# RaphaelHaddad/Real-Time-Brain-Inspired-Video-Memory

Hardware: NVIDIA B200
Metric: queries_per_sec_top10_384d (higher is better)
Workload: dtype tf32

## Files before the change

include/vidmem.h:

```cpp
#ifndef VIDMEM_H_
#define VIDMEM_H_

#include <stddef.h>
#include <stdint.h>

#ifdef __cplusplus
extern "C" {
#endif

#define VM_ABI_VERSION 1

typedef enum vm_status {
    VM_OK = 0,
    VM_ERR_BADARG = -1,
    VM_ERR_OOM = -2,
    VM_ERR_CUDA = -3,
    VM_ERR_NCCL = -4,
    VM_ERR_OVERFLOW = -5,
    VM_ERR_UNSUPPORTED = -6,
    VM_ERR_STATE = -7
} vm_status;

typedef enum vm_dtype { VM_F32 = 0, VM_BF16 = 1, VM_F64 = 2 } vm_dtype;
typedef enum vm_mem { VM_MEM_HOST = 0, VM_MEM_DEVICE = 1 } vm_mem;

typedef enum vm_score_mode { VM_SCORE_RAW = 0, VM_SCORE_NEO4J = 1 } vm_score_mode;

typedef enum vm_sum_mode { VM_SUM_NAIVE = 0, VM_SUM_NEUMAIER = 1 } vm_sum_mode;

enum {
    VM_FLAG_ASYNC = 1,
    VM_FLAG_FORCE_EXACT = 2,
    VM_FLAG_FORCE_SIMT = 4,
    VM_FLAG_FORCE_TC = 8,
    VM_FLAG_TIMING = 16,
    VM_FLAG_NO_SPLIT = 32,
    VM_FLAG_SPLIT = 64
};

typedef struct vm_store vm_store;
typedef struct vm_comm vm_comm;

typedef struct vm_topk_stats {
    int32_t scan_kernel;
    int32_t scan_launches;
    int32_t uncertified;
    int32_t candidates;
    int32_t scan_ctas;
    int32_t scan_stages;
    int32_t full_rescans;
    int32_t scan_variant;
} vm_topk_stats;

int vm_version(void);
const char *vm_last_error(void);
int vm_device_info(int device, int *sm_count, int *cc_major, int *cc_minor, size_t *total_mem);

int vm_store_create(vm_store **out, int device, int dim, int dtype, int64_t capacity);
int vm_store_attach(vm_store **out, int device, int dim, int dtype, int64_t capacity, void *rows_dev,
                    float *inv_norms_dev);
int vm_store_create_exact(vm_store **out, int device, int dim, int shadow_dtype, int64_t capacity);
int vm_store_attach_exact(vm_store **out, int device, int dim, int shadow_dtype, int64_t capacity, void *rows_dev,
                          float *inv_norms_dev, double *rows_exact_dev);
int vm_store_create_growable(vm_store **out, int device, int dim, int dtype, int exact, int64_t initial_capacity,
                             int64_t max_capacity);
int vm_store_reserve(vm_store *s, int64_t capacity);
int64_t vm_store_max_capacity(const vm_store *s);
size_t vm_store_resident_bytes(const vm_store *s);
void *vm_store_rows_ptr(const vm_store *s);
float *vm_store_inv_norms_ptr(const vm_store *s);
double *vm_store_rows_exact_ptr(const vm_store *s);
int vm_store_destroy(vm_store *s);
int64_t vm_store_size(const vm_store *s);
int64_t vm_store_capacity(const vm_store *s);
int vm_store_dim(const vm_store *s);
int vm_store_ld(const vm_store *s);
int vm_ld(int dim);

int vm_store_append(vm_store *s, const void *rows, int src_dtype, int src_mem, int64_t n, int64_t *first_row,
                    void *stream);
int vm_store_update(vm_store *s, int64_t row0, const void *rows, int src_dtype, int src_mem, int64_t n,
                    void *stream);
int vm_store_invalidate(vm_store *s, const int64_t *rows_host, int64_t n, void *stream);
int vm_store_set_size(vm_store *s, int64_t n, int64_t recompute_from_row, void *stream);
int vm_store_clear(vm_store *s);
int vm_store_last_scan_ms(vm_store *s, float *ms);
int vm_store_avg_scan_ms(vm_store *s, float *ms, int *calls);

typedef struct vm_store_counters {
    int64_t batches;
    int64_t queries;
    int64_t uncertified;
    int64_t band_settled;
    int64_t collect_settled;
    int64_t full_rescans;
    int64_t bound_violations;
} vm_store_counters;
int vm_store_read_counters(vm_store *s, vm_store_counters *out, int reset);

int vm_store_band_keys(vm_store *s, int nq_cap, int64_t *kept_per_query, int64_t *spilled_per_query, int *nq_out);

int vm_topk(vm_store *s, const void *queries, int q_dtype, int q_mem, int nq, int k, double min_score,
            int score_mode, int sum_mode, int flags, int64_t *out_idx, double *out_score, int32_t *out_count,
            int out_mem, vm_topk_stats *stats, void *stream);

int vm_topk_sharded(vm_store *s, vm_comm *comm, int64_t row_offset, const void *queries, int q_dtype, int q_mem,
                    int nq, int k, double min_score, int score_mode, int sum_mode, int flags, int64_t *out_idx,
                    double *out_score, int32_t *out_count, int out_mem, vm_topk_stats *stats, void *stream);

int vm_merge_topk_lists(int device, const int64_t *idx_dev, const double *score_dev, const int32_t *count_dev,
                        int nlists, int nq, int k, int64_t *out_idx_dev, double *out_score_dev,
                        int32_t *out_count_dev, void *stream);

size_t vm_topk_packed_bytes(int nq, int k);
int vm_merge_topk_packed(int device, const void *packed_dev, int nlists, int nq, int k, int64_t *out_idx_dev,
                         double *out_score_dev, int32_t *out_count_dev, void *stream);

int vm_merge_max_by_id(int device, const int64_t *idx_dev, const double *score_dev, const int32_t *count_dev,
                       int nq, int k, int k2, int64_t *out_idx_dev, double *out_score_dev,
                       int32_t *out_count_dev, void *stream);

int vm_cosine_pairs(int device, const void *a, const void *b, int dtype, int mem, int64_t n, int dim, int zero_rule,
                    int sum_mode, double *out, int out_mem, void *stream);

int vm_pairs_above(int device, const void *x_dev, int dtype, int64_t n, int dim, float threshold, int64_t cap,
                   int64_t *out_i_dev, int64_t *out_j_dev, float *out_score_dev, int64_t *out_count_dev, int part,
                   int nparts, int flags, void *stream);

int vm_pairs_above_sharded(vm_comm *comm, void *x_dev, int dtype, int64_t n, int dim, float threshold, int64_t cap,
                           int64_t *out_i_dev, int64_t *out_j_dev, float *out_score_dev, int64_t *out_count_dev,
                           int root, int flags, void *stream);

int vm_comm_unique_id(void *out128);
int vm_comm_init_rank(vm_comm **out, int device, int nranks, int rank, const void *id128);
int vm_comm_destroy(vm_comm *c);
size_t vm_comm_exchange_bytes(void);
int vm_comm_attach_peer_buffers(vm_comm *c, void *const *bufs, int nranks);
int vm_comm_nranks(const vm_comm *c);
int vm_comm_rank(const vm_comm *c);

int vm_synth_fill(int device, void *rows_dev, int dtype, uint64_t seed, int64_t row0, int64_t n, int dim,
                  uint64_t dup_period, void *stream);

#ifdef __cplusplus
}
#endif
#endif
```

real-time-brain-inspired-video-memory_b200/_lib.py:

```python
from __future__ import annotations

import ctypes as C
import os
import sys

HERE = os.path.dirname(os.path.abspath(__file__))
LIB_PATH = os.environ.get("VIDMEM_LIB", os.path.join(HERE, "libvidmem.so"))

VM_OK = 0
VM_ERR_BADARG, VM_ERR_OOM, VM_ERR_CUDA, VM_ERR_NCCL, VM_ERR_OVERFLOW, VM_ERR_UNSUPPORTED, VM_ERR_STATE = -1, -2, -3, -4, -5, -6, -7
VM_F32, VM_BF16, VM_F64 = 0, 1, 2
VM_MEM_HOST, VM_MEM_DEVICE = 0, 1
VM_SCORE_RAW, VM_SCORE_NEO4J = 0, 1
VM_SUM_NAIVE, VM_SUM_NEUMAIER = 0, 1
VM_FLAG_ASYNC, VM_FLAG_FORCE_EXACT, VM_FLAG_FORCE_SIMT, VM_FLAG_FORCE_TC, VM_FLAG_TIMING, VM_FLAG_NO_SPLIT, VM_FLAG_SPLIT = 1, 2, 4, 8, 16, 32, 64

DEFAULT_SUM_MODE = VM_SUM_NEUMAIER if sys.version_info >= (3, 12) else VM_SUM_NAIVE

EXPORTS = [
    "vm_version", "vm_last_error", "vm_device_info", "vm_ld",
    "vm_store_create", "vm_store_attach", "vm_store_create_exact", "vm_store_attach_exact", "vm_store_create_growable", "vm_store_reserve",
    "vm_store_max_capacity", "vm_store_resident_bytes", "vm_store_rows_ptr", "vm_store_inv_norms_ptr", "vm_store_rows_exact_ptr", "vm_store_destroy", "vm_store_size", "vm_store_capacity", "vm_store_dim",
    "vm_store_ld", "vm_store_append", "vm_store_update", "vm_store_invalidate", "vm_store_set_size", "vm_store_clear",
    "vm_store_last_scan_ms",
    "vm_store_avg_scan_ms", "vm_store_read_counters", "vm_store_band_keys",
    "vm_topk", "vm_topk_sharded", "vm_merge_topk_lists", "vm_topk_packed_bytes", "vm_merge_topk_packed", "vm_merge_max_by_id", "vm_cosine_pairs", "vm_pairs_above", "vm_pairs_above_sharded",
    "vm_comm_unique_id", "vm_comm_init_rank", "vm_comm_destroy", "vm_comm_exchange_bytes", "vm_comm_attach_peer_buffers", "vm_comm_nranks", "vm_comm_rank", "vm_synth_fill",
]


class TopkStats(C.Structure):
    _fields_ = [("scan_kernel", C.c_int32), ("scan_launches", C.c_int32), ("uncertified", C.c_int32),
                ("candidates", C.c_int32), ("scan_ctas", C.c_int32), ("scan_stages", C.c_int32), ("full_rescans", C.c_int32), ("scan_variant", C.c_int32)]


class StoreCounters(C.Structure):
    _fields_ = [(n, C.c_int64) for n in ("batches", "queries", "uncertified", "band_settled", "collect_settled", "full_rescans", "bound_violations")]

    def as_dict(self):
        return {n: int(getattr(self, n)) for n, _ in self._fields_}


class VidmemError(RuntimeError):
    def __init__(self, code: int, msg: str):
        super().__init__(f"libvidmem error {code}: {msg}")
        self.code = code


_lib = None


def load() -> C.CDLL:
    global _lib
    if _lib is not None:
        return _lib
    if not os.path.exists(LIB_PATH):
        if os.environ.get("VIDMEM_BUILD") == "1":
            from . import build as _build
            _build.build()
        else:
            raise ImportError(f"{LIB_PATH} is missing: build it with `python {HERE}/build.py` "
                              "(there is no CPU fallback)")
    L = C.CDLL(LIB_PATH)
    vp, i64, i32, dbl = C.c_void_p, C.c_int64, C.c_int32, C.c_double
    ci, u64, sz = C.c_int, C.c_uint64, C.c_size_t
    P = C.POINTER
    sig = {
        "vm_version": (ci, []),
        "vm_last_error": (C.c_char_p, []),
        "vm_device_info": (ci, [ci, P(ci), P(ci), P(ci), P(sz)]),
        "vm_ld": (ci, [ci]),
        "vm_store_create": (ci, [P(vp), ci, ci, ci, i64]),
        "vm_store_attach": (ci, [P(vp), ci, ci, ci, i64, vp, vp]),
        "vm_store_create_exact": (ci, [P(vp), ci, ci, ci, i64]),
        "vm_store_attach_exact": (ci, [P(vp), ci, ci, ci, i64, vp, vp, vp]),
        "vm_store_create_growable": (ci, [P(vp), ci, ci, ci, ci, i64, i64]),
        "vm_store_reserve": (ci, [vp, i64]),
        "vm_store_max_capacity": (i64, [vp]),
        "vm_store_resident_bytes": (sz, [vp]),
        "vm_store_rows_ptr": (vp, [vp]),
        "vm_store_inv_norms_ptr": (vp, [vp]),
        "vm_store_rows_exact_ptr": (vp, [vp]),
        "vm_store_destroy": (ci, [vp]),
        "vm_store_size": (i64, [vp]),
        "vm_store_capacity": (i64, [vp]),
        "vm_store_dim": (ci, [vp]),
        "vm_store_ld": (ci, [vp]),
        "vm_store_append": (ci, [vp, vp, ci, ci, i64, P(i64), vp]),
        "vm_store_update": (ci, [vp, i64, vp, ci, ci, i64, vp]),
        "vm_store_invalidate": (ci, [vp, vp, i64, vp]),
        "vm_store_set_size": (ci, [vp, i64, i64, vp]),
        "vm_store_clear": (ci, [vp]),
        "vm_store_last_scan_ms": (ci, [vp, P(C.c_float)]),
        "vm_store_avg_scan_ms": (ci, [vp, P(C.c_float), P(C.c_int)]),
        "vm_store_read_counters": (ci, [vp, P(StoreCounters), ci]),
        "vm_store_band_keys": (ci, [vp, ci, P(i64), P(i64), P(ci)]),
        "vm_topk": (ci, [vp, vp, ci, ci, ci, ci, dbl, ci, ci, ci, vp, vp, vp, ci, P(TopkStats), vp]),
        "vm_topk_sharded": (ci, [vp, vp, i64, vp, ci, ci, ci, ci, dbl, ci, ci, ci, vp, vp, vp, ci, P(TopkStats), vp]),
        "vm_merge_topk_lists": (ci, [ci, vp, vp, vp, ci, ci, ci, vp, vp, vp, vp]),
        "vm_topk_packed_bytes": (sz, [ci, ci]),
        "vm_merge_topk_packed": (ci, [ci, vp, ci, ci, ci, vp, vp, vp, vp]),
        "vm_merge_max_by_id": (ci, [ci, vp, vp, vp, ci, ci, ci, vp, vp, vp, vp]),
        "vm_cosine_pairs": (ci, [ci, vp, vp, ci, ci, i64, ci, ci, ci, vp, ci, vp]),
        "vm_pairs_above": (ci, [ci, vp, ci, i64, ci, C.c_float, i64, vp, vp, vp, vp, ci, ci, ci, vp]),
        "vm_pairs_above_sharded": (ci, [vp, vp, ci, i64, ci, C.c_float, i64, vp, vp, vp, vp, ci, ci, vp]),
        "vm_comm_unique_id": (ci, [vp]),
        "vm_comm_init_rank": (ci, [P(vp), ci, ci, ci, vp]),
        "vm_comm_destroy": (ci, [vp]),
        "vm_comm_exchange_bytes": (sz, []),
        "vm_comm_attach_peer_buffers": (ci, [vp, P(vp), ci]),
        "vm_comm_nranks": (ci, [vp]),
        "vm_comm_rank": (ci, [vp]),
        "vm_synth_fill": (ci, [ci, vp, ci, u64, i64, i64, ci, u64, vp]),
    }
    for name, (res, args) in sig.items():
        f = getattr(L, name)
        f.restype, f.argtypes = res, args
    if L.vm_version() != 1:
        raise ImportError("libvidmem ABI version mismatch")
    _lib = L
    return L


def check(rc: int, allow=()) -> int:
    if rc != VM_OK and rc not in allow:
        msg = load().vm_last_error()
        raise VidmemError(rc, msg.decode("utf-8", "replace") if msg else "")
    return rc
```

real-time-brain-inspired-video-memory_b200/csrc/api.cu:

```cuda
#include "common.cuh"

#include <dlfcn.h>
#include <stdarg.h>
#include <stdlib.h>
#include <string.h>
#include <time.h>
#include <new>
#include <vector>

namespace vm {

static thread_local char g_err[512] = "";
void set_error(const char *fmt, ...)
{
    va_list ap;
    va_start(ap, fmt);
    vsnprintf(g_err, sizeof(g_err), fmt, ap);
    va_end(ap);
}

int k_convert_rows(const void *src, int src_dtype, void *dst, int dst_dtype, int64_t n, int dim, int ld, cudaStream_t st);
int k_row_inv_norms(const void *rows, int dtype, float *inv_norms, int64_t row0, int64_t n, int ld, int *extreme, cudaStream_t st,
                    const double *exact = nullptr);
int k_invalidate_rows(float *inv_norms, const int64_t *rows_dev, int64_t n, int64_t size, cudaStream_t st);
int k_normalize_queries(const void *q, int q_dtype, int nq, int nq_pad, int dim, int ld, float *out_f32, void *out_bf16,
                        int32_t *zero_me, uint32_t *zero_tab, int zero_tab_n, int tf32_round, int split, bool pdl, cudaStream_t st);
int k_synth_fill(void *rows, int dtype, uint64_t seed, int64_t row0, int64_t n, int dim, int ld, uint64_t dup_period,
                 cudaStream_t st);
int k_merge_candidates(const uint64_t *cand, int lists, int nq, int kp, uint64_t *merged, cudaStream_t st);

int k_slab_top(const SelectArgs &sa, int nq, int kp, uint64_t *merged, int *incomplete, cudaStream_t st);
int k_rescore(const RescoreArgs &a, cudaStream_t st, const int *incomplete);
int k_select_rescore(const SelectArgs &sa, const RescoreArgs &a, cudaStream_t st, bool pdl);
bool select_rescore_fits(int lists, int list_len, int kp, int dtype, int dim, int ld);
int k_collect_rescore(const uint64_t *buf, const int *cnt, int cap, const RescoreArgs &a, cudaStream_t st);
int k_exact(const ExactArgs &a, cudaStream_t st, bool pdl);
int k_merge_topk_lists(const void *idx, const void *score, const void *count, size_t stride_bytes, int lists, int nq, int k,
                       int64_t *out_idx, double *out_score, int32_t *out_count, cudaStream_t st);
int k_p2p_publish(void *flag, unsigned long long gen, cudaStream_t st);
int k_merge_topk_p2p(void *const *peers, int nranks, size_t slot_off, size_t flag_off, unsigned long long gen, int nq, int k,
                     int64_t *out_idx, double *out_score, int32_t *out_count, cudaStream_t st);
int k_merge_max_by_id(const int64_t *idx, const double *score, const int32_t *count, int nq, int k, int k2,
                      int64_t *out_idx, double *out_score, int32_t *out_count, cudaStream_t st);
int k_cosine_pairs(const void *a, const void *b, int dtype, int64_t n, int dim, int zero_rule, int sum_mode, double *out,
                   cudaStream_t st);
int k_pairs_above(int device, const void *x, int dtype, int64_t n, int dim, int ld, float threshold, int64_t cap,
                  int64_t *out_i, int64_t *out_j, float *out_score, int64_t *out_count, int part, int nparts, int flags,
                  cudaStream_t st);
int k_pairs_concat(const void *gathered, size_t per_rank_bytes, int64_t slot, const int64_t *counts, int nranks, int64_t cap,
                   int64_t *out_i, int64_t *out_j, float *out_score, int64_t *out_count, cudaStream_t st);

struct Arena;
int arena_create(Arena **out, int device, size_t max_bytes);
int arena_grow(Arena *a, size_t bytes);
void arena_destroy(Arena *a);
void *arena_base(const Arena *a);
size_t arena_mapped(const Arena *a);

static constexpr int MAXQ = 64;
static constexpr int MAXK = 64;
static constexpr int XCTAS = 148;
static constexpr int MAX_DEVICES = 64;
static constexpr int COLLECT_CAP = 4096;
static constexpr int FLAG_INTERNAL_CAPTURE = 1 << 30;

struct ResultBlock {
    int64_t *idx;
    double *score;
    int32_t *count;
    static ResultBlock at(void *base, int nq, int k)
    {
        char *b = (char *)base;
        return {(int64_t *)b, (double *)(b + (size_t)nq * k * 8), (int32_t *)(b + (size_t)nq * k * 16)};
    }
    ResultBlock from(int q0, int k) const { return {idx + (size_t)q0 * k, score + (size_t)q0 * k, count + q0}; }
};
static constexpr size_t result_bytes(int nq, int k) { return (size_t)nq * k * 16 + (size_t)nq * 4; }
static constexpr size_t packed_bytes(int nq, int k) { return (result_bytes(nq, k) + 7) & ~(size_t)7; }

static void unpack_to_host(const void *pack, int nq, int k, const ResultBlock &out)
{
    const ResultBlock p = ResultBlock::at(const_cast<void *>(pack), nq, k);
    memcpy(out.idx, p.idx, (size_t)nq * k * 8);
    memcpy(out.score, p.score, (size_t)nq * k * 8);
    memcpy(out.count, p.count, (size_t)nq * 4);
}

struct DeviceGuard {
    int prev = -1;
    bool ok = true;
    explicit DeviceGuard(int dev)
    {
        if (cudaGetDevice(&prev) != cudaSuccess) { ok = false; return; }
        if (prev != dev && cudaSetDevice(dev) != cudaSuccess) ok = false;
    }
    ~DeviceGuard() { if (prev >= 0) cudaSetDevice(prev); }
};

struct Buf {
    void *p = nullptr;
    size_t bytes = 0;
    int ensure(size_t need)
    {
        if (need <= bytes) return VM_OK;
        if (p) cudaFree(p);
        p = nullptr; bytes = 0;
        cudaError_t e = cudaMalloc(&p, need);
        if (e != cudaSuccess) { set_error("cudaMalloc(%zu) failed: %s", need, cudaGetErrorString(e)); return VM_ERR_OOM; }
        bytes = need;
        return VM_OK;
    }
    void release() { if (p) cudaFree(p); p = nullptr; bytes = 0; }
};

struct Workspace {
    bool ready = false;
    int lists_max = 0;
    Buf q_raw, q_f32, q_bf16, seed, cand, merged, o_idx, flags, col_thr, col_cnt, col_buf, xs, xr, xc, taken, gather_send, gather_recv, misc, ubuf, done, scnt, sel_inc;
    int32_t *h_uncert = nullptr;
    unsigned char *h_pack = nullptr;
    unsigned char *h_q = nullptr;
    void release()
    {
        Buf *all[] = {&q_raw, &q_f32, &q_bf16, &seed, &cand, &merged, &o_idx, &flags, &col_thr, &col_cnt, &col_buf, &xs, &xr, &xc, &taken,
                      &gather_send, &gather_recv, &misc, &ubuf, &done, &scnt, &sel_inc};
        for (Buf *b : all) b->release();
        if (h_uncert) cudaFreeHost(h_uncert);
        if (h_pack) cudaFreeHost(h_pack);
        if (h_q) cudaFreeHost(h_q);
        h_uncert = nullptr; h_pack = nullptr; h_q = nullptr;
        ready = false;
    }
};

}

using namespace vm;

struct vm_store {
    int device = 0, dim = 0, ld = 0, dtype = VM_F32, sm_count = 148;
    int64_t capacity = 0, size = 0;
    void *rows = nullptr;
    float *inv_norms = nullptr;
    double *rows_exact = nullptr;
    bool owns = false;
    Arena *ar_rows = nullptr, *ar_inv = nullptr, *ar_exact = nullptr;
    int64_t max_capacity = 0;
    const void *exact_rows() const { return rows_exact ? (const void *)rows_exact : (const void *)rows; }
    int exact_dtype() const { return rows_exact ? (int)VM_F64 : dtype; }
    int *extreme = nullptr;
    unsigned long long *cum = nullptr;
    int64_t n_batches = 0, n_queries = 0;
    int last_band_ctas = 0, last_band_nq = 0;
    Buf stage, stage_idx;
    Workspace ws;
    static constexpr int EV_RING = 64;
    cudaEvent_t evr[EV_RING][2] = {};
    int ev_next = 0;
    int ev_pending = 0;
    int ev_cur = -1;
    bool timed = false;
    struct GraphEntry {
        cudaGraphExec_t exec = nullptr;
        uint64_t version = 0;
        int nq = 0, k = 0, flags = 0, score_mode = 0, sum_mode = 0, q_dtype = 0;
        double min_score = 0.0;
        int64_t row_offset = 0;
        vm_topk_stats stats{};
    };
    GraphEntry graphs[4];
    int graph_next = 0;
    uint64_t version = 1;
    uint64_t seen_version = 0;
    int stable_calls = 0;
    cudaStream_t gstream = nullptr;
};

static constexpr size_t XCHG_SLOT_BYTES = (result_bytes(MAXQ, MAXK) + 255) & ~(size_t)255;
static constexpr size_t XCHG_FLAG_OFF = 2 * XCHG_SLOT_BYTES;
static constexpr size_t XCHG_BYTES = XCHG_FLAG_OFF + 256;

struct vm_comm {
    void *nccl = nullptr;
    int nranks = 1, rank = 0, device = 0;
    void *peer[16] = {};
    bool p2p = false;
    unsigned long long gen = 0;
    Buf pl_i, pl_j, pl_s, pl_cnt, pg_cnt, pg_send, pg_recv;
    int64_t *h_counts = nullptr;
};

struct Id128 { char b[128]; };
namespace {
struct NcclApi {
    void *h = nullptr;
    int (*GetUniqueId)(void *) = nullptr;
    int (*CommInitRank)(void **, int,  Id128, int) = nullptr;
    int (*AllGather)(const void *, void *, size_t, int, void *, cudaStream_t) = nullptr;
    int (*Broadcast)(const void *, void *, size_t, int, int, void *, cudaStream_t) = nullptr;
    int (*CommDestroy)(void *) = nullptr;
    const char *(*GetErrorString)(int) = nullptr;
};
}
static NcclApi g_nccl;

static int nccl_load()
{
    if (g_nccl.h) return VM_OK;
    void *h = dlopen("libnccl.so.2", RTLD_NOW | RTLD_GLOBAL);
    if (!h) h = dlopen("libnccl.so", RTLD_NOW | RTLD_GLOBAL);
    VM_REQUIRE(h, VM_ERR_NCCL, "cannot load libnccl.so.2: %s", dlerror());
    g_nccl.GetUniqueId = (int (*)(void *))dlsym(h, "ncclGetUniqueId");
    g_nccl.CommInitRank = (int (*)(void **, int, Id128, int))dlsym(h, "ncclCommInitRank");
    g_nccl.AllGather = (int (*)(const void *, void *, size_t, int, void *, cudaStream_t))dlsym(h, "ncclAllGather");
    g_nccl.Broadcast = (int (*)(const void *, void *, size_t, int, int, void *, cudaStream_t))dlsym(h, "ncclBroadcast");
    g_nccl.CommDestroy = (int (*)(void *))dlsym(h, "ncclCommDestroy");
    g_nccl.GetErrorString = (const char *(*)(int))dlsym(h, "ncclGetErrorString");
    VM_REQUIRE(g_nccl.GetUniqueId && g_nccl.CommInitRank && g_nccl.AllGather && g_nccl.Broadcast && g_nccl.CommDestroy, VM_ERR_NCCL,
               "libnccl lacks a required symbol");
    g_nccl.h = h;
    return VM_OK;
}
#define VM_NCCL_CHECK(expr)                                                                            \
    do {                                                                                               \
        int _r = (expr);                                                                               \
        if (_r != 0) {                                                                                 \
            set_error("%s failed: %s", #expr, g_nccl.GetErrorString ? g_nccl.GetErrorString(_r) : "?"); \
            return VM_ERR_NCCL;                                                                        \
        }                                                                                              \
    } while (0)

static int check_arch(int device, int *sm_count)
{
    cudaDeviceProp p;
    VM_CUDA_CHECK(cudaGetDeviceProperties(&p, device));
    VM_REQUIRE(p.major == 10, VM_ERR_UNSUPPORTED, "device %d is sm_%d%d; libvidmem is built for sm_100a only", device,
               p.major, p.minor);
    if (sm_count) *sm_count = p.multiProcessorCount;
    return VM_OK;
}

static int ws_prepare(vm_store *s)
{
    Workspace &w = s->ws;
    if (w.ready) return VM_OK;
    int lists = 2 * s->sm_count;
    w.lists_max = lists;
    int rc;
#define ENS(b, bytes) if ((rc = (b).ensure(bytes)) != VM_OK) return rc
    ENS(w.q_raw, (size_t)MAXQ * s->dim * 8);
    ENS(w.q_f32, (size_t)MAXQ * s->ld * 4);
    ENS(w.q_bf16, (size_t)2 * MAXQ * s->ld * 2);
    ENS(w.cand, (size_t)lists * MAXQ * (MAXK > SCAN_SLAB ? MAXK : SCAN_SLAB) * 8);
    ENS(w.merged, (size_t)MAXQ * MAXK * 8);
    ENS(w.o_idx, result_bytes(MAXQ, MAXK) + 64);
    ENS(w.flags, (size_t)(MAXQ + 2) * 4);
    ENS(w.seed, (size_t)(SEED_TAB_WORDS + 3 * MAXQ) * 4);
    ENS(w.ubuf, (size_t)MAXQ * SCAN_UNION_CAP * 8);
    ENS(w.done, 64);
    ENS(w.scnt, (size_t)256 * MAXQ * 4);
    ENS(w.sel_inc, (size_t)MAXQ * 4);
    VM_CUDA_CHECK(cudaMemset(w.done.p, 0, 64));
    ENS(w.col_thr, (size_t)MAXQ * 4);
    ENS(w.col_cnt, (size_t)MAXQ * 4);
    ENS(w.col_buf, (size_t)MAXQ * COLLECT_CAP * 8);
    ENS(w.xs, (size_t)XCTAS * MAXQ * MAXK * 8);
    ENS(w.xr, (size_t)XCTAS * MAXQ * MAXK * 4);
    ENS(w.xc, (size_t)XCTAS * MAXQ * 4);
    ENS(w.taken, (size_t)MAXQ * XCTAS * MAXK);
#undef ENS
    VM_CUDA_CHECK(cudaMallocHost((void **)&w.h_uncert, 64));
    VM_CUDA_CHECK(cudaMallocHost((void **)&w.h_pack, result_bytes(MAXQ, MAXK) + 64));
    VM_CUDA_CHECK(cudaMallocHost((void **)&w.h_q, (size_t)MAXQ * s->dim * 8));
    w.ready = true;
    return VM_OK;
}

static double scan_eps_stored(int kernel, int store_dtype, int dim, int split);
static double scan_eps(int kernel, int store_dtype, int dim, int split, bool shadow = false)
{
    const double base = scan_eps_stored(kernel, store_dtype, dim, split);
    if (!shadow) return base;
    return base + (store_dtype == VM_F32 ? 1.1920928955078125e-07 : 1.953125e-3 * 1.01);
}
static double scan_eps_stored(int kernel, int store_dtype, int dim, int split)
{
    const double u = 1.1920928955078125e-07;
    const double fp32_acc = (double)(dim + 16) * u;
    if (kernel == 1) return fp32_acc;
    if (store_dtype == VM_F32)
        return 9.765625e-4 + 4.8828125e-4 + 1e-6 + fp32_acc;
    if (!split) return 3.90625e-3 + fp32_acc;
    return 1.52587890625e-5 * 1.01 + (double)(dim + dim / 8 + 32) * u;
}

extern "C" int vm_version(void) { return VM_ABI_VERSION; }
extern "C" const char *vm_last_error(void) { return g_err; }

extern "C" int vm_device_info(int device, int *sm_count, int *cc_major, int *cc_minor, size_t *total_mem)
{
    cudaDeviceProp p;
    VM_CUDA_CHECK(cudaGetDeviceProperties(&p, device));
    if (sm_count) *sm_count = p.multiProcessorCount;
    if (cc_major) *cc_major = p.major;
    if (cc_minor) *cc_minor = p.minor;
    if (total_mem) *total_mem = p.totalGlobalMem;
    return VM_OK;
}

extern "C" int vm_ld(int dim) { return ld_for_dim(dim); }

static int store_new(vm_store **out, int device, int dim, int dtype, int64_t capacity)
{
    VM_REQUIRE(out, VM_ERR_BADARG, "out is NULL");
    VM_REQUIRE(dim >= 1 && dim <= 4096, VM_ERR_BADARG, "dim %d outside [1, 4096]", dim);
    VM_REQUIRE(dtype == VM_F32 || dtype == VM_BF16, VM_ERR_BADARG, "store dtype must be VM_F32 or VM_BF16");
    VM_REQUIRE(capacity >= 1 && capacity < 0xFFFFFFFFLL, VM_ERR_BADARG, "capacity %lld outside [1, 2^32-2]", (long long)capacity);
    int sms = 0;
    int rc = check_arch(device, &sms);
    if (rc != VM_OK) return rc;
    vm_store *s = new (std::nothrow) vm_store();
    VM_REQUIRE(s, VM_ERR_OOM, "host allocation failed");
    s->device = device; s->dim = dim; s->ld = ld_for_dim(dim); s->dtype = dtype; s->capacity = capacity; s->sm_count = sms;
    {
        DeviceGuard g(device);
        if (cudaMalloc((void **)&s->extreme, 4) != cudaSuccess || cudaMemset(s->extreme, 0, 4) != cudaSuccess ||
            cudaMalloc((void **)&s->cum, 64) != cudaSuccess || cudaMemset(s->cum, 0, 64) != cudaSuccess) {
            set_error("store allocation failed");
            vm_store_destroy(s);
            return VM_ERR_OOM;
        }
    }
    *out = s;
    return VM_OK;
}

extern "C" int vm_store_create(vm_store **out, int device, int dim, int dtype, int64_t capacity)
{
    int rc = store_new(out, device, dim, dtype, capacity);
    if (rc != VM_OK) return rc;
    vm_store *s = *out;
    DeviceGuard g(device);
    s->owns = true;
    size_t bytes = (size_t)capacity * s->ld * dtype_size(dtype);
    cudaError_t e = cudaMalloc(&s->rows, bytes);
    if (e == cudaSuccess) e = cudaMalloc((void **)&s->inv_norms, (size_t)capacity * 4);
    if (e != cudaSuccess) {
        set_error("store allocation of %zu bytes failed: %s", bytes, cudaGetErrorString(e));
        vm_store_destroy(s);
        *out = nullptr;
        return VM_ERR_OOM;
    }
    return VM_OK;
}

extern "C" int vm_store_create_exact(vm_store **out, int device, int dim, int shadow_dtype, int64_t capacity)
{
    int rc = vm_store_create(out, device, dim, shadow_dtype, capacity);
    if (rc != VM_OK) return rc;
    vm_store *s = *out;
    DeviceGuard g(device);
    const size_t bytes = (size_t)capacity * s->ld * 8;
    cudaError_t e = cudaMalloc((void **)&s->rows_exact, bytes);
    if (e != cudaSuccess) {
        set_error("store allocation of %zu bytes (binary64 rows) failed: %s", bytes, cudaGetErrorString(e));
        vm_store_destroy(s);
        *out = nullptr;
        return VM_ERR_OOM;
    }
    return VM_OK;
}

static int store_back(vm_store *s, int64_t capacity)
{
    int rc = arena_grow(s->ar_rows, (size_t)capacity * s->ld * dtype_size(s->dtype));
    if (rc == VM_OK) rc = arena_grow(s->ar_inv, (size_t)capacity * 4);
    if (rc == VM_OK && s->ar_exact) rc = arena_grow(s->ar_exact, (size_t)capacity * s->ld * 8);
    return rc;
}

extern "C" int vm_store_create_growable(vm_store **out, int device, int dim, int dtype, int exact, int64_t initial_capacity,
                                        int64_t max_capacity)
{
    VM_REQUIRE(initial_capacity >= 1 && max_capacity >= initial_capacity, VM_ERR_BADARG, "need 1 <= initial_capacity <= max_capacity");
    int rc = store_new(out, device, dim, dtype, max_capacity);
    if (rc != VM_OK) return rc;
    vm_store *s = *out;
    DeviceGuard g(device);
    s->max_capacity = max_capacity;
    s->capacity = initial_capacity;
    rc = arena_create(&s->ar_rows, device, (size_t)max_capacity * s->ld * dtype_size(dtype));
    if (rc == VM_OK) rc = arena_create(&s->ar_inv, device, (size_t)max_capacity * 4);
    if (rc == VM_OK && exact) rc = arena_create(&s->ar_exact, device, (size_t)max_capacity * s->ld * 8);
    if (rc == VM_OK) rc = store_back(s, initial_capacity);
    if (rc != VM_OK) { vm_store_destroy(s); *out = nullptr; return rc; }
    s->rows = arena_base(s->ar_rows);
    s->inv_norms = (float *)arena_base(s->ar_inv);
    if (exact) s->rows_exact = (double *)arena_base(s->ar_exact);
    return VM_OK;
}

extern "C" int vm_store_reserve(vm_store *s, int64_t capacity)
{
    VM_REQUIRE(s, VM_ERR_BADARG, "store is NULL");
    if (capacity <= s->capacity) return VM_OK;
    VM_REQUIRE(s->ar_rows, VM_ERR_STATE, "store is not growable (created over fixed buffers of %lld rows)", (long long)s->capacity);
    VM_REQUIRE(capacity <= s->max_capacity, VM_ERR_OVERFLOW, "capacity %lld exceeds the reserved maximum %lld", (long long)capacity,
               (long long)s->max_capacity);
    DeviceGuard g(s->device);
    int rc = store_back(s, capacity);
    if (rc != VM_OK) return rc;
    s->capacity = capacity;
    return VM_OK;
}

extern "C" int64_t vm_store_max_capacity(const vm_store *s) { return s ? (s->ar_rows ? s->max_capacity : s->capacity) : -1; }
extern "C" void *vm_store_rows_ptr(const vm_store *s) { return s ? s->rows : nullptr; }
extern "C" float *vm_store_inv_norms_ptr(const vm_store *s) { return s ? s->inv_norms : nullptr; }
extern "C" double *vm_store_rows_exact_ptr(const vm_store *s) { return s ? s->rows_exact : nullptr; }
extern "C" size_t vm_store_resident_bytes(const vm_store *s)
{
    if (!s) return 0;
    if (s->ar_rows) return arena_mapped(s->ar_rows) + arena_mapped(s->ar_inv) + (s->ar_exact ? arena_mapped(s->ar_exact) : 0);
    return (size_t)s->capacity * ((size_t)s->ld * (dtype_size(s->dtype) + (s->rows_exact ? 8 : 0)) + 4);
}

extern "C" int vm_store_attach_exact(vm_store **out, int device, int dim, int shadow_dtype, int64_t capacity, void *rows_dev,
                                     float *inv_norms_dev, double *rows_exact_dev)
{
    VM_REQUIRE(rows_exact_dev && ((uintptr_t)rows_exact_dev & 15) == 0, VM_ERR_BADARG, "binary64 rows buffer must be 16-byte aligned");
    int rc = vm_store_attach(out, device, dim, shadow_dtype, capacity, rows_dev, inv_norms_dev);
    if (rc != VM_OK) return rc;
    (*out)->rows_exact = rows_exact_dev;
    return VM_OK;
}

extern "C" int vm_store_attach(vm_store **out, int device, int dim, int dtype, int64_t capacity, void *rows_dev,
                               float *inv_norms_dev)
{
    VM_REQUIRE(rows_dev && inv_norms_dev, VM_ERR_BADARG, "attach needs device buffers");
    VM_REQUIRE(((uintptr_t)rows_dev & 127) == 0, VM_ERR_BADARG, "rows buffer must be 128-byte aligned");
    int rc = store_new(out, device, dim, dtype, capacity);
    if (rc != VM_OK) return rc;
    (*out)->rows = rows_dev;
    (*out)->inv_norms = inv_norms_dev;
    (*out)->owns = false;
    return VM_OK;
}

extern "C" int vm_store_destroy(vm_store *s)
{
    if (!s) return VM_OK;
    DeviceGuard g(s->device);
    cudaDeviceSynchronize();
    if (s->owns) { cudaFree(s->rows); cudaFree(s->inv_norms); if (s->rows_exact) cudaFree(s->rows_exact); }
    arena_destroy(s->ar_rows); arena_destroy(s->ar_inv); arena_destroy(s->ar_exact);
    if (s->extreme) cudaFree(s->extreme);
    if (s->cum) cudaFree(s->cum);
    s->stage.release(); s->stage_idx.release();
    s->ws.release();
    for (auto &pr : s->evr) { if (pr[0]) cudaEventDestroy(pr[0]); if (pr[1]) cudaEventDestroy(pr[1]); }
    for (auto &ge : s->graphs) if (ge.exec) cudaGraphExecDestroy(ge.exec);
    if (s->gstream) cudaStreamDestroy(s->gstream);
    delete s;
    return VM_OK;
}

extern "C" int64_t vm_store_size(const vm_store *s) { return s ? s->size : -1; }
extern "C" int64_t vm_store_capacity(const vm_store *s) { return s ? s->capacity : -1; }
extern "C" int vm_store_dim(const vm_store *s) { return s ? s->dim : -1; }
extern "C" int vm_store_ld(const vm_store *s) { return s ? s->ld : -1; }

static int store_write(vm_store *s, int64_t row0, const void *rows, int src_dtype, int src_mem, int64_t n, cudaStream_t st)
{
    VM_REQUIRE(src_dtype == VM_F32 || src_dtype == VM_BF16 || src_dtype == VM_F64, VM_ERR_BADARG, "bad source dtype");
    if (n == 0) return VM_OK;
    VM_REQUIRE(rows, VM_ERR_BADARG, "rows is NULL");
    DeviceGuard g(s->device);
    const void *src = rows;
    if (src_mem == VM_MEM_HOST) {
        size_t bytes = (size_t)n * s->dim * dtype_size(src_dtype);
        int rc = s->stage.ensure(bytes);
        if (rc != VM_OK) return rc;
        VM_CUDA_CHECK(cudaMemcpyAsync(s->stage.p, rows, bytes, cudaMemcpyHostToDevice, st));
        src = s->stage.p;
    }
    char *dst = (char *)s->rows + (size_t)row0 * s->ld * dtype_size(s->dtype);
    int rc = k_convert_rows(src, src_dtype, dst, s->dtype, n, s->dim, s->ld, st);
    if (rc != VM_OK) return rc;
    if (s->rows_exact) {
        rc = k_convert_rows(src, src_dtype, s->rows_exact + (size_t)row0 * s->ld, VM_F64, n, s->dim, s->ld, st);
        if (rc != VM_OK) return rc;
    }
    return k_row_inv_norms(s->rows, s->dtype, s->inv_norms, row0, row0 + n, s->ld, s->extreme, st, s->rows_exact);
}

extern "C" int vm_store_append(vm_store *s, const void *rows, int src_dtype, int src_mem, int64_t n, int64_t *first_row,
                               void *stream)
{
    VM_REQUIRE(s, VM_ERR_BADARG, "store is NULL");
    VM_REQUIRE(n >= 0, VM_ERR_BADARG, "n < 0");
    if (s->ar_rows && s->size + n > s->capacity) {
        const int64_t row_bytes = (int64_t)s->ld * (int64_t)(dtype_size(s->dtype) + (s->rows_exact ? 8 : 0)) + 4;
        const int64_t slack_rows = ((int64_t)256 << 20) / row_bytes + 1;
        int64_t want = s->size + n + slack_rows;
        if (want > s->max_capacity) want = s->max_capacity;
        if (want >= s->size + n) {
            int rc = vm_store_reserve(s, want);
            if (rc != VM_OK && want > s->size + n) rc = vm_store_reserve(s, s->size + n);
            if (rc != VM_OK) return rc;
        }
    }
    VM_REQUIRE(s->size + n <= s->capacity, VM_ERR_OVERFLOW, "append of %lld rows exceeds capacity %lld (size %lld)",
               (long long)n, (long long)s->capacity, (long long)s->size);
    int rc = store_write(s, s->size, rows, src_dtype, src_mem, n, (cudaStream_t)stream);
    if (rc != VM_OK) return rc;
    if (first_row) *first_row = s->size;
    s->size += n;
    ++s->version;
    return VM_OK;
}

extern "C" int vm_store_update(vm_store *s, int64_t row0, const void *rows, int src_dtype, int src_mem, int64_t n, void *stream)
{
    VM_REQUIRE(s, VM_ERR_BADARG, "store is NULL");
    VM_REQUIRE(row0 >= 0 && n >= 0 && row0 + n <= s->size, VM_ERR_BADARG, "update range [%lld, %lld) outside [0, %lld)",
               (long long)row0, (long long)(row0 + n), (long long)s->size);
    ++s->version;
    return store_write(s, row0, rows, src_dtype, src_mem, n, (cudaStream_t)stream);
}

extern "C" int vm_store_invalidate(vm_store *s, const int64_t *rows_host, int64_t n, void *stream)
{
    VM_REQUIRE(s, VM_ERR_BADARG, "store is NULL");
    if (n <= 0) return VM_OK;
    VM_REQUIRE(rows_host, VM_ERR_BADARG, "rows is NULL");
    DeviceGuard g(s->device);
    int rc = s->stage_idx.ensure((size_t)n * 8);
    if (rc != VM_OK) return rc;
    VM_CUDA_CHECK(cudaMemcpyAsync(s->stage_idx.p, rows_host, (size_t)n * 8, cudaMemcpyHostToDevice, (cudaStream_t)stream));
    ++s->version;
    return k_invalidate_rows(s->inv_norms, (const int64_t *)s->stage_idx.p, n, s->size, (cudaStream_t)stream);
}

extern "C" int vm_store_set_size(vm_store *s, int64_t n, int64_t recompute_from_row, void *stream)
{
    VM_REQUIRE(s, VM_ERR_BADARG, "store is NULL");
    VM_REQUIRE(n >= 0 && n <= s->capacity, VM_ERR_BADARG, "size %lld outside [0, capacity]", (long long)n);
    DeviceGuard g(s->device);
    s->size = n;
    ++s->version;
    if (recompute_from_row >= 0 && recompute_from_row < n) {
        if (s->rows_exact) {
            const int64_t r0 = recompute_from_row;
            int rc = k_convert_rows((const char *)s->rows + (size_t)r0 * s->ld * dtype_size(s->dtype), s->dtype,
                                    s->rows_exact + (size_t)r0 * s->ld, VM_F64, n - r0, s->ld, s->ld, (cudaStream_t)stream);
            if (rc != VM_OK) return rc;
        }
        return k_row_inv_norms(s->rows, s->dtype, s->inv_norms, recompute_from_row, n, s->ld, s->extreme, (cudaStream_t)stream, s->rows_exact);
    }
    return VM_OK;
}

extern "C" int vm_store_last_scan_ms(vm_store *s, float *ms)
{
    VM_REQUIRE(s && ms, VM_ERR_BADARG, "NULL argument");
    VM_REQUIRE(s->timed, VM_ERR_STATE, "no vm_topk call with VM_FLAG_TIMING has run the scan kernel yet");
    DeviceGuard g(s->device);
    VM_CUDA_CHECK(cudaEventSynchronize(s->evr[s->ev_cur][1]));
    VM_CUDA_CHECK(cudaEventElapsedTime(ms, s->evr[s->ev_cur][0], s->evr[s->ev_cur][1]));
    return VM_OK;
}

extern "C" int vm_store_avg_scan_ms(vm_store *s, float *ms, int *calls)
{
    VM_REQUIRE(s && ms, VM_ERR_BADARG, "NULL argument");
    VM_REQUIRE(s->timed && s->ev_pending > 0, VM_ERR_STATE, "no vm_topk call with VM_FLAG_TIMING since the last read");
    DeviceGuard g(s->device);
    VM_CUDA_CHECK(cudaEventSynchronize(s->evr[s->ev_cur][1]));
    double sum = 0.0;
    const int n = s->ev_pending;
    for (int i = 0; i < n; ++i) {
        const int slot = (s->ev_cur - i + 2 * vm_store::EV_RING) % vm_store::EV_RING;
        float t = 0.0f;
        VM_CUDA_CHECK(cudaEventElapsedTime(&t, s->evr[slot][0], s->evr[slot][1]));
        sum += t;
    }
    *ms = (float)(sum / n);
    if (calls) *calls = n;
    s->ev_pending = 0;
    return VM_OK;
}

extern "C" int vm_store_band_keys(vm_store *s, int nq_cap, int64_t *kept_per_query, int64_t *spilled_per_query, int *nq_out)
{
    VM_REQUIRE(s && kept_per_query && spilled_per_query, VM_ERR_BADARG, "NULL argument");
    VM_REQUIRE(s->ws.ready && s->last_band_ctas > 0, VM_ERR_STATE, "the last top-k call of this store was not a band-keeping tcgen05 scan");
    const int ctas = s->last_band_ctas, nq = s->last_band_nq;
    VM_REQUIRE(nq_cap >= nq, VM_ERR_BADARG, "room for %d queries needed", nq);
    DeviceGuard g(s->device);
    VM_CUDA_CHECK(cudaDeviceSynchronize());
    std::vector<int> sc((size_t)ctas * nq), uc(nq);
    VM_CUDA_CHECK(cudaMemcpy(sc.data(), s->ws.scnt.p, sc.size() * 4, cudaMemcpyDeviceToHost));
    VM_CUDA_CHECK(cudaMemcpy(uc.data(), (int *)s->ws.seed.p + SEED_TAB_WORDS + 2 * MAXQ, (size_t)nq * 4, cudaMemcpyDeviceToHost));
    for (int q = 0; q < nq; ++q) {
        int64_t k = 0;
        for (int c = 0; c < ctas; ++c) k += sc[(size_t)c * nq + q];
        kept_per_query[q] = k;
        spilled_per_query[q] = uc[q];
    }
    if (nq_out) *nq_out = nq;
    return VM_OK;
}

extern "C" int vm_store_read_counters(vm_store *s, vm_store_counters *out, int reset)
{
    VM_REQUIRE(s && out, VM_ERR_BADARG, "NULL argument");
    DeviceGuard g(s->device);
    unsigned long long h[8] = {0, 0, 0, 0, 0, 0, 0, 0};
    VM_CUDA_CHECK(cudaMemcpy(h, s->cum, sizeof(h), cudaMemcpyDeviceToHost));
    out->batches = s->n_batches; out->queries = s->n_queries;
    out->uncertified = (int64_t)h[0]; out->band_settled = (int64_t)h[1]; out->collect_settled = (int64_t)h[2];
    out->full_rescans = (int64_t)h[3];
    out->bound_violations = (int64_t)h[4];
    if (reset) {
        VM_CUDA_CHECK(cudaMemset(s->cum, 0, sizeof(h)));
        s->n_batches = 0; s->n_queries = 0;
    }
    return VM_OK;
}

extern "C" int vm_store_clear(vm_store *s)
{
    VM_REQUIRE(s, VM_ERR_BADARG, "store is NULL");
    DeviceGuard g(s->device);
    VM_CUDA_CHECK(cudaMemset(s->extreme, 0, 4));
    s->size = 0;
    ++s->version;
    return VM_OK;
}

extern "C" size_t vm_topk_packed_bytes(int nq, int k) { return nq > 0 && k > 0 ? packed_bytes(nq, k) : 0; }

namespace {
struct TopkCall {
    vm_store *s;
    const void *queries;
    int q_dtype, q_mem, nq, k;
    double min_score;
    int score_mode, sum_mode, flags;
    int64_t row_offset;
    ResultBlock d;
    cudaStream_t st;
    vm_topk_stats *stats;
    ResultBlock h = {};
};
}

static cudaError_t wait_stream(cudaStream_t st, const vm_store *s = nullptr)
{
    static const bool block = [] { const char *e = getenv("VIDMEM_SYNC"); return e && !strcmp(e, "block"); }();
    if (block) return cudaStreamSynchronize(st);
    if (s) {
        const double est_us = (double)s->size * s->ld * (double)dtype_size(s->dtype) / 6.5e6;
        if (est_us > 400.0) {
            struct timespec ts;
            const long ns = (long)(est_us * 750.0);
            ts.tv_sec = ns / 1000000000L; ts.tv_nsec = ns % 1000000000L;
            nanosleep(&ts, nullptr);
        }
    }
    for (;;) {
        const cudaError_t e = cudaStreamQuery(st);
        if (e != cudaErrorNotReady) return e;
#if defined(__x86_64__) || defined(__i386__)
        __builtin_ia32_pause();
#endif
    }
}

static int pack_out_enqueue(const TopkCall &c)
{
    VM_CUDA_CHECK(cudaMemcpyAsync(c.s->ws.h_pack, c.d.idx, result_bytes(c.nq, c.k), cudaMemcpyDeviceToHost, c.st));
    return VM_OK;
}

static int tc_list_len(int k) { return k <= 16 ? 32 : (k <= 48 ? 64 : 0); }

static int queries_per_pass(const vm_store *s, int k, int flags)
{
    const int kp = tc_list_len(k);
    if (!(flags & (VM_FLAG_FORCE_EXACT | VM_FLAG_FORCE_SIMT)) && kp)
        for (int nq = 64; nq >= 16; nq -= 16)
            if (scan_tc_supported(s->dtype, s->dim, nq, kp)) return nq;
    return MAXQ;
}

static int topk_batch(const TopkCall &c)
{
    vm_store *s = c.s;
    Workspace &w = s->ws;
    cudaStream_t st = c.st;
    const void *q_dev = c.queries;
    if (c.q_mem == VM_MEM_HOST) {
        const size_t qbytes = (size_t)c.nq * s->dim * dtype_size(c.q_dtype);
        memcpy(w.h_q, c.queries, qbytes);
        VM_CUDA_CHECK(cudaMemcpyAsync(w.q_raw.p, w.h_q, qbytes, cudaMemcpyHostToDevice, st));
        q_dev = w.q_raw.p;
    }
    FinalizeArgs fin{c.k, c.min_score, c.score_mode, c.row_offset, c.d.idx, c.d.score, c.d.count};
    ExactArgs ex{s->exact_rows(), s->inv_norms, s->exact_dtype(), s->ld, s->dim, s->size, q_dev, c.q_dtype, c.nq, c.k, c.sum_mode,
                 nullptr, (double *)w.xs.p, (uint32_t *)w.xr.p, (int32_t *)w.xc.p, (uint8_t *)w.taken.p, XCTAS, fin, s->cum,
                 (int *)w.done.p};
    if (!(c.flags & FLAG_INTERNAL_CAPTURE)) { ++s->n_batches; s->n_queries += c.nq; }
    int launches = 0;
    if (c.stats) { c.stats->uncertified = 0; c.stats->candidates = 0; c.stats->scan_ctas = 0; }

    int kernel = 0, kp = 0;
    if (!(c.flags & VM_FLAG_FORCE_EXACT) && s->size > 0) {
        int kp_tc = tc_list_len(c.k);
        int kp_simt = c.k <= 24 ? (c.k + 8 > 16 ? ((c.k + 8 + 7) & ~7) : 16) : 0;
        bool tc_ok = kp_tc > 0 && scan_tc_supported(s->dtype, s->dim, c.nq, kp_tc);
        bool want_tc = !(c.flags & VM_FLAG_FORCE_SIMT);
        if (want_tc && tc_ok) { kernel = 2; kp = kp_tc; }
        else if (kp_simt > 0) { kernel = 1; kp = kp_simt; }
        else if (tc_ok) { kernel = 2; kp = kp_tc; }
    }
    if (kernel == 0) {
        int rc = k_exact(ex, st, false);
        if (rc != VM_OK) return rc;
        launches += 2;
        if (c.h.idx) {
            if ((rc = pack_out_enqueue(c)) != VM_OK) return rc;
            VM_CUDA_CHECK(wait_stream(st, s));
            unpack_to_host(w.h_pack, c.nq, c.k, c.h);
        }
        if (c.stats) { c.stats->scan_kernel = 0; c.stats->scan_launches += launches; }
        return VM_OK;
    }

    int nq_pad = kernel == 2 ? ((c.nq + 15) & ~15) : c.nq;
    const int split = (kernel == 2 && s->dtype == VM_BF16 && !(c.flags & VM_FLAG_NO_SPLIT) &&
                       (c.nq <= 48 || (c.flags & VM_FLAG_SPLIT)) && scan_tc_supported(s->dtype, s->dim, c.nq, kp, 1)) ? 1 : 0;
#ifdef VIDMEM_NO_GRAPH_PDL
    const bool pdl = !(c.flags & (VM_FLAG_TIMING | FLAG_INTERNAL_CAPTURE));
#else
    const bool pdl = !(c.flags & VM_FLAG_TIMING);
#endif
    int rc = k_normalize_queries(q_dev, c.q_dtype, c.nq, nq_pad, s->dim, s->ld, (float *)w.q_f32.p,
                                 (kernel == 2 && s->dtype == VM_BF16) ? w.q_bf16.p : nullptr,
                                 (int32_t *)w.flags.p + c.nq, kernel == 2 ? (uint32_t *)w.seed.p : nullptr,
                                 kernel == 2 ? (int)(w.seed.bytes / 4) : 0, kernel == 2 && s->dtype == VM_F32, split, pdl, st);
    if (rc != VM_OK) return rc;
    ++launches;
    const double eps = scan_eps(kernel, s->dtype, s->dim, split, s->rows_exact != nullptr);

    ScanArgs a;
    ScanInfo sinfo;
    a.rows = s->rows; a.inv_norms = s->inv_norms; a.dtype = s->dtype; a.n = s->size; a.dim = s->dim; a.ld = s->ld;
    a.queries = (const float *)w.q_f32.p; a.nq = c.nq; a.kp = kp; a.cand = (uint64_t *)w.cand.p; a.stream = st;
    a.slab = (uint64_t *)w.cand.p; a.scnt = (int *)w.scnt.p;
    a.ubuf = (uint64_t *)w.ubuf.p; a.ucnt = (int *)w.seed.p + SEED_TAB_WORDS + 2 * MAXQ; a.ucap = SCAN_UNION_CAP;
    a.band = nextafterf((float)(2.0 * eps), INFINITY); a.ksel = c.k; a.split = split; a.pdl = pdl;
    const bool timing = (c.flags & VM_FLAG_TIMING) != 0;
    if (timing) {
        s->ev_cur = s->ev_next;
        s->ev_next = (s->ev_next + 1) % vm_store::EV_RING;
        if (s->ev_pending < vm_store::EV_RING) ++s->ev_pending;
        if (!s->evr[s->ev_cur][0]) { VM_CUDA_CHECK(cudaEventCreate(&s->evr[s->ev_cur][0])); VM_CUDA_CHECK(cudaEventCreate(&s->evr[s->ev_cur][1])); }
        VM_CUDA_CHECK(cudaEventRecord(s->evr[s->ev_cur][0], st));
    }
    if (kernel == 1) {
        int64_t need = (s->size + 31) / 32;
        a.ctas = (int)imin64(need, 2 * s->sm_count);
        rc = launch_scan_simt(a);
        launches += (c.nq + 7) / 8;
    } else {
        int64_t tiles = (s->size + 127) / 128;
        a.ctas = (int)imin64(tiles, s->sm_count);

        a.dump = tiles <= s->sm_count && tiles * SCAN_DUMP_TILE <= SCAN_DUMP_MAX_KEYS &&
                 (size_t)tiles * c.nq * SCAN_DUMP_TILE * 8 <= w.cand.bytes &&
                 select_rescore_fits((int)tiles, SCAN_DUMP_TILE, kp, s->exact_dtype(), s->dim, s->ld);
        s->last_band_ctas = a.dump ? 0 : a.ctas; s->last_band_nq = c.nq;
        rc = launch_scan_tc(a, s->dtype == VM_BF16 ? w.q_bf16.p : w.q_f32.p, (uint32_t *)w.seed.p, (int *)w.flags.p + c.nq + 1, nullptr, &sinfo);
        launches += 1;
    }
    if (rc != VM_OK) return rc;
    if (timing) { VM_CUDA_CHECK(cudaEventRecord(s->evr[s->ev_cur][1], st)); s->timed = true; }

    int32_t *flags = (int32_t *)w.flags.p;
    int32_t *uncert = flags + c.nq;
    RescoreArgs rs{(const uint64_t *)w.merged.p, kp, s->exact_rows(), s->inv_norms, s->exact_dtype(), s->ld, s->dim, s->size, q_dev,
                   c.q_dtype, c.nq, eps, c.sum_mode, fin, flags, uncert, s->extreme,
                   kernel == 2 ? (float *)w.col_thr.p : nullptr, s->cum};
    SelectArgs sel;
    const bool union_src = kernel == 2 && !a.dump;
    if (union_src) {
        sel.slab = a.slab; sel.scnt = a.scnt; sel.ctas = a.ctas; sel.ubuf = a.ubuf; sel.ucnt = a.ucnt; sel.ucap = a.ucap;
        sel.seed_tab = a.ctas <= 256 ? (const uint32_t *)w.seed.p : nullptr; sel.nq_pad = nq_pad; sel.ksel = c.k; sel.band = a.band;
    } else { sel.cand = a.cand; sel.lists = a.ctas; sel.list_len = a.dump ? SCAN_DUMP_TILE : kp; sel.complete = a.dump ? 1 : 0; }
    rc = k_select_rescore(sel, rs, st, pdl);
    if (rc == VM_ERR_UNSUPPORTED && !a.dump) {
        if (union_src) rc = k_slab_top(sel, c.nq, kp, (uint64_t *)w.merged.p, (int *)w.sel_inc.p, st);
        else rc = k_merge_candidates(a.cand, a.ctas, c.nq, kp, (uint64_t *)w.merged.p, st);
        if (rc != VM_OK) return rc;
        rc = k_rescore(rs, st, union_src ? (const int *)w.sel_inc.p : nullptr);
        ++launches;
    }
    if (rc != VM_OK) return rc;
    launches += 1;

    ex.flags = flags;
    int n_uncert = 0, n_full = -1;
    auto run_collect = [&]() -> int {
        VM_CUDA_CHECK(cudaMemsetAsync(w.col_cnt.p, 0, (size_t)c.nq * 4, st));
        ScanCollect sc{(const float *)w.col_thr.p, (uint64_t *)w.col_buf.p, (int *)w.col_cnt.p, COLLECT_CAP, uncert};
        int r = launch_scan_tc(a, s->dtype == VM_BF16 ? w.q_bf16.p : w.q_f32.p, nullptr, nullptr, &sc);
        if (r != VM_OK) return r;
        return k_collect_rescore((const uint64_t *)w.col_buf.p, (const int *)w.col_cnt.p, COLLECT_CAP, rs, st);
    };
    if (c.flags & VM_FLAG_ASYNC) {
        if (c.flags & FLAG_INTERNAL_CAPTURE) {
            VM_CUDA_CHECK(cudaMemcpyAsync(w.h_uncert, uncert, 4, cudaMemcpyDeviceToHost, st));
        } else {
            rc = k_exact(ex, st, pdl);
            if (rc != VM_OK) return rc;
            launches += 1;
        }
        n_uncert = -1;
    } else {
        VM_CUDA_CHECK(cudaMemcpyAsync(w.h_uncert, uncert, 4, cudaMemcpyDeviceToHost, st));
        if (c.h.idx && (rc = pack_out_enqueue(c)) != VM_OK) return rc;
        VM_CUDA_CHECK(wait_stream(st, s));
        n_uncert = *w.h_uncert;
        n_full = 0;
        if (n_uncert > 0) {
            int left = n_uncert;
            if (kernel == 2) {
                if ((rc = run_collect()) != VM_OK) return rc;
                launches += 2;
                VM_CUDA_CHECK(cudaMemcpyAsync(w.h_uncert, uncert, 4, cudaMemcpyDeviceToHost, st));
                VM_CUDA_CHECK(wait_stream(st, s));
                left = *w.h_uncert;
            }
            n_full = left;
            if (left > 0) {
                rc = k_exact(ex, st, false);
                if (rc != VM_OK) return rc;
                launches += 1;
            }
            if (c.h.idx) {
                if ((rc = pack_out_enqueue(c)) != VM_OK) return rc;
                VM_CUDA_CHECK(wait_stream(st, s));
            }
        }
        if (c.h.idx) unpack_to_host(w.h_pack, c.nq, c.k, c.h);
    }
    if (c.stats) {
        c.stats->scan_kernel = kernel;
        c.stats->scan_launches += launches;
        c.stats->uncertified += n_uncert > 0 ? n_uncert : 0;
        c.stats->full_rescans = n_full;
        c.stats->candidates = kp;
        c.stats->scan_ctas = a.ctas;
        c.stats->scan_stages = kernel == 2 ? sinfo.stages : 0;
        c.stats->scan_variant = kernel == 2 ? sinfo.variant : 0;
    }
    return VM_OK;
}

static constexpr int GRAPH_SKIPPED = 1;

static int graph_capture(const TopkCall &c, vm_store::GraphEntry *ge)
{
    vm_store *s = c.s;
    Workspace &w = s->ws;
    vm_topk_stats cs{};
    TopkCall cc = c;
    cc.queries = w.q_raw.p; cc.q_mem = VM_MEM_DEVICE; cc.flags |= VM_FLAG_ASYNC | FLAG_INTERNAL_CAPTURE;
    cc.d = ResultBlock::at(w.o_idx.p, c.nq, c.k); cc.st = s->gstream; cc.stats = &cs;
    const size_t qbytes = (size_t)c.nq * s->dim * dtype_size(c.q_dtype);
    cudaGraph_t graph = nullptr;
    VM_CUDA_CHECK(cudaStreamBeginCapture(s->gstream, cudaStreamCaptureModeRelaxed));
    int rc = VM_OK;
    if (cudaMemcpyAsync(w.q_raw.p, w.h_q, qbytes, cudaMemcpyHostToDevice, s->gstream) != cudaSuccess) rc = VM_ERR_CUDA;
    if (rc == VM_OK) rc = topk_batch(cc);
    if (rc == VM_OK && cudaMemcpyAsync(w.h_pack, cc.d.idx, result_bytes(c.nq, c.k), cudaMemcpyDeviceToHost, s->gstream) != cudaSuccess)
        rc = VM_ERR_CUDA;
    cudaError_t ce = cudaStreamEndCapture(s->gstream, &graph);
    if (rc != VM_OK || ce != cudaSuccess || !graph) {
        if (graph) cudaGraphDestroy(graph);
        if (rc == VM_OK) { set_error("graph capture failed: %s", cudaGetErrorString(ce)); rc = VM_ERR_CUDA; }
        cudaGetLastError();
        return rc;
    }
    ce = cudaGraphInstantiate(&ge->exec, graph, 0);
    cudaGraphDestroy(graph);
    if (ce != cudaSuccess) { ge->exec = nullptr; set_error("cudaGraphInstantiate failed: %s", cudaGetErrorString(ce)); return VM_ERR_CUDA; }
    ge->version = s->version; ge->nq = c.nq; ge->k = c.k; ge->flags = c.flags; ge->score_mode = c.score_mode;
    ge->sum_mode = c.sum_mode; ge->q_dtype = c.q_dtype; ge->min_score = c.min_score; ge->row_offset = c.row_offset; ge->stats = cs;
    return VM_OK;
}

static int topk_graph(const TopkCall &c, int out_mem, bool sharded, const ResultBlock &out)
{
    vm_store *s = c.s;
    Workspace &w = s->ws;
    static const bool no_graph = getenv("VIDMEM_NO_GRAPH") != nullptr;
    if (s->seen_version == s->version) { if (s->stable_calls < 1 << 20) ++s->stable_calls; }
    else { s->seen_version = s->version; s->stable_calls = 0; }
    if (no_graph || s->stable_calls < 16 || sharded || c.st != nullptr || c.q_mem != VM_MEM_HOST || out_mem != VM_MEM_HOST ||
        (c.flags & (VM_FLAG_ASYNC | VM_FLAG_TIMING | VM_FLAG_FORCE_EXACT)) || s->size == 0 ||
        c.nq > queries_per_pass(s, c.k, c.flags))
        return GRAPH_SKIPPED;
    if (!s->gstream) VM_CUDA_CHECK(cudaStreamCreate(&s->gstream));
    vm_store::GraphEntry *ge = nullptr;
    for (auto &e : s->graphs)
        if (e.exec && e.version == s->version && e.nq == c.nq && e.k == c.k && e.flags == c.flags && e.score_mode == c.score_mode &&
            e.sum_mode == c.sum_mode && e.q_dtype == c.q_dtype && e.row_offset == c.row_offset &&
            memcmp(&e.min_score, &c.min_score, sizeof(double)) == 0) { ge = &e; break; }
    if (!ge) {
        ge = &s->graphs[s->graph_next];
        s->graph_next = (s->graph_next + 1) & 3;
        if (ge->exec) { cudaGraphExecDestroy(ge->exec); ge->exec = nullptr; }
        const int rc = graph_capture(c, ge);
        if (rc != VM_OK) return rc;
    }
    memcpy(w.h_q, c.queries, (size_t)c.nq * s->dim * dtype_size(c.q_dtype));
    ++s->n_batches; s->n_queries += c.nq;
    VM_CUDA_CHECK(cudaGraphLaunch(ge->exec, s->gstream));
    VM_CUDA_CHECK(wait_stream(s->gstream, s));
    const int uncertified = ge->stats.scan_kernel != 0 ? *w.h_uncert : 0;
    if (uncertified > 0) {
        TopkCall rerun = c;
        rerun.d = ResultBlock::at(w.o_idx.p, c.nq, c.k); rerun.st = s->gstream; rerun.h = out;
        return topk_batch(rerun);
    }
    unpack_to_host(w.h_pack, c.nq, c.k, out);
    if (c.stats) { *c.stats = ge->stats; c.stats->uncertified = uncertified; }
    return VM_OK;
}

static size_t xchg_slot_off(unsigned long long gen) { return (size_t)(gen & 1) * XCHG_SLOT_BYTES; }

static ResultBlock batch_dest(vm_store *s, const vm_comm *comm, bool sharded, int out_mem, const ResultBlock &out, int nb, int k)
{
    if (sharded && comm->p2p) return ResultBlock::at((char *)comm->peer[comm->rank] + xchg_slot_off(comm->gen), nb, k);
    if (sharded) return ResultBlock::at(s->ws.gather_send.p, nb, k);
    return out_mem == VM_MEM_DEVICE ? out : ResultBlock::at(s->ws.o_idx.p, nb, k);
}

static int exchange_merge(vm_store *s, vm_comm *comm, int nb, int k, const ResultBlock &m, cudaStream_t st)
{
    if (comm->p2p) {
        const int rc = k_p2p_publish((char *)comm->peer[comm->rank] + XCHG_FLAG_OFF, comm->gen, st);
        if (rc != VM_OK) return rc;
        return k_merge_topk_p2p(comm->peer, comm->nranks, xchg_slot_off(comm->gen), XCHG_FLAG_OFF, comm->gen, nb, k, m.idx, m.score,
                                m.count, st);
    }
    const Workspace &w = s->ws;
    VM_NCCL_CHECK(g_nccl.AllGather(w.gather_send.p, w.gather_recv.p, packed_bytes(nb, k),  0, comm->nccl, st));
    const ResultBlock r = ResultBlock::at(w.gather_recv.p, nb, k);
    return k_merge_topk_lists(r.idx, r.score, r.count, packed_bytes(nb, k), comm->nranks, nb, k, m.idx, m.score, m.count, st);
}

static int topk_common(vm_store *s, vm_comm *comm, int64_t row_offset, const void *queries, int q_dtype, int q_mem, int nq,
                       int k, double min_score, int score_mode, int sum_mode, int flags, int64_t *out_idx,
                       double *out_score, int32_t *out_count, int out_mem, vm_topk_stats *stats, void *stream)
{
    VM_REQUIRE(s, VM_ERR_BADARG, "store is NULL");
    VM_REQUIRE(nq >= 0, VM_ERR_BADARG, "nq < 0");
    VM_REQUIRE(k >= 1 && k <= MAXK, VM_ERR_BADARG, "k %d outside [1, %d]", k, MAXK);
    VM_REQUIRE(q_dtype == VM_F32 || q_dtype == VM_BF16 || q_dtype == VM_F64, VM_ERR_BADARG, "bad query dtype");
    VM_REQUIRE(score_mode == VM_SCORE_RAW || score_mode == VM_SCORE_NEO4J, VM_ERR_BADARG, "bad score_mode");
    VM_REQUIRE(sum_mode == VM_SUM_NAIVE || sum_mode == VM_SUM_NEUMAIER, VM_ERR_BADARG, "bad sum_mode");
    VM_REQUIRE(!(flags & VM_FLAG_ASYNC) || (out_mem == VM_MEM_DEVICE && q_mem == VM_MEM_DEVICE), VM_ERR_BADARG,
               "VM_FLAG_ASYNC needs device queries and device outputs");
    if (stats) memset(stats, 0, sizeof(*stats));
    if (nq == 0) return VM_OK;
    VM_REQUIRE(queries && out_idx && out_score && out_count, VM_ERR_BADARG, "NULL buffer");
    DeviceGuard g(s->device);
    VM_REQUIRE(g.ok, VM_ERR_CUDA, "cannot select device %d", s->device);
    int rc = ws_prepare(s);
    if (rc != VM_OK) return rc;
    const bool sharded = comm && comm->nranks > 1;
    const ResultBlock out{out_idx, out_score, out_count};
    const TopkCall call{s, queries, q_dtype, q_mem, nq, k, min_score, score_mode, sum_mode, flags, row_offset, {}, (cudaStream_t)stream,
                        stats};
    if ((rc = topk_graph(call, out_mem, sharded, out)) != GRAPH_SKIPPED) return rc;

    Workspace &w = s->ws;
    const int bq = queries_per_pass(s, k, flags);
    for (int q0 = 0; q0 < nq; q0 += bq) {
        const int nb = nq - q0 < bq ? nq - q0 : bq;
        const ResultBlock out_b = out.from(q0, k);
        if (sharded && comm->p2p) {
            ++comm->gen;
        } else if (sharded) {
            if ((rc = w.gather_send.ensure(packed_bytes(nb, k))) != VM_OK) return rc;
            if ((rc = w.gather_recv.ensure(packed_bytes(nb, k) * comm->nranks)) != VM_OK) return rc;
        }
        TopkCall c = call;
        c.queries = (const char *)queries + (size_t)q0 * s->dim * dtype_size(q_dtype);
        c.nq = nb;
        c.d = batch_dest(s, comm, sharded, out_mem, out_b, nb, k);
        if (out_mem == VM_MEM_HOST) {
            if (sharded) c.flags |= VM_FLAG_ASYNC;
            else c.h = out_b;
        }
        if ((rc = topk_batch(c)) != VM_OK) return rc;
        if (!sharded) continue;
        const ResultBlock ws = ResultBlock::at(w.o_idx.p, nb, k);
        if ((rc = exchange_merge(s, comm, nb, k, out_mem == VM_MEM_DEVICE ? out_b : ws, c.st)) != VM_OK) return rc;
        if (stats) stats->scan_launches += 2;
        if (out_mem == VM_MEM_HOST) {
            VM_CUDA_CHECK(cudaMemcpyAsync(w.h_pack, ws.idx, result_bytes(nb, k), cudaMemcpyDeviceToHost, c.st));
            VM_CUDA_CHECK(wait_stream(c.st, s));
            unpack_to_host(w.h_pack, nb, k, out_b);
        }
    }
    return VM_OK;
}

extern "C" int vm_topk(vm_store *s, const void *queries, int q_dtype, int q_mem, int nq, int k, double min_score,
                       int score_mode, int sum_mode, int flags, int64_t *out_idx, double *out_score, int32_t *out_count,
                       int out_mem, vm_topk_stats *stats, void *stream)
{
    return topk_common(s, nullptr, 0, queries, q_dtype, q_mem, nq, k, min_score, score_mode, sum_mode, flags, out_idx,
                       out_score, out_count, out_mem, stats, stream);
}

extern "C" int vm_topk_sharded(vm_store *s, vm_comm *comm, int64_t row_offset, const void *queries, int q_dtype, int q_mem,
                               int nq, int k, double min_score, int score_mode, int sum_mode, int flags, int64_t *out_idx,
                               double *out_score, int32_t *out_count, int out_mem, vm_topk_stats *stats, void *stream)
{
    VM_REQUIRE(comm, VM_ERR_BADARG, "comm is NULL");
    return topk_common(s, comm, row_offset, queries, q_dtype, q_mem, nq, k, min_score, score_mode, sum_mode, flags, out_idx,
                       out_score, out_count, out_mem, stats, stream);
}

extern "C" int vm_merge_topk_lists(int device, const int64_t *idx_dev, const double *score_dev, const int32_t *count_dev,
                                   int nlists, int nq, int k, int64_t *out_idx_dev, double *out_score_dev,
                                   int32_t *out_count_dev, void *stream)
{
    VM_REQUIRE(idx_dev && score_dev && count_dev && out_idx_dev && out_score_dev && out_count_dev, VM_ERR_BADARG, "NULL buffer");
    VM_REQUIRE(nlists >= 1 && nq >= 1 && k >= 1, VM_ERR_BADARG, "bad shape");
    DeviceGuard g(device);
    size_t stride = (size_t)nq * k * 8;
    VM_REQUIRE(device >= 0 && device < MAX_DEVICES, VM_ERR_BADARG, "device index %d outside [0, %d)", device, MAX_DEVICES);
    static thread_local Buf cnt_wide_dev[MAX_DEVICES];
    Buf &cnt_wide = cnt_wide_dev[device];
    int rc = cnt_wide.ensure(stride * nlists);
    if (rc != VM_OK) return rc;
    VM_CUDA_CHECK(cudaMemcpy2DAsync(cnt_wide.p, stride, count_dev, (size_t)nq * 4, (size_t)nq * 4, nlists,
                                    cudaMemcpyDeviceToDevice, (cudaStream_t)stream));
    return k_merge_topk_lists(idx_dev, score_dev, cnt_wide.p, stride, nlists, nq, k, out_idx_dev, out_score_dev,
                              out_count_dev, (cudaStream_t)stream);
}

extern "C" int vm_merge_topk_packed(int device, const void *packed_dev, int nlists, int nq, int k, int64_t *out_idx_dev,
                                    double *out_score_dev, int32_t *out_count_dev, void *stream)
{
    VM_REQUIRE(packed_dev && out_idx_dev && out_score_dev && out_count_dev, VM_ERR_BADARG, "NULL buffer");
    VM_REQUIRE(nlists >= 1 && nq >= 1 && k >= 1, VM_ERR_BADARG, "bad shape");
    DeviceGuard g(device);
    const ResultBlock r = ResultBlock::at(const_cast<void *>(packed_dev), nq, k);
    return k_merge_topk_lists(r.idx, r.score, r.count, packed_bytes(nq, k), nlists, nq, k, out_idx_dev, out_score_dev,
                              out_count_dev, (cudaStream_t)stream);
}

extern "C" int vm_merge_max_by_id(int device, const int64_t *idx_dev, const double *score_dev, const int32_t *count_dev,
                                  int nq, int k, int k2, int64_t *out_idx_dev, double *out_score_dev, int32_t *out_count_dev,
                                  void *stream)
{
    VM_REQUIRE(idx_dev && score_dev && count_dev && out_idx_dev && out_score_dev && out_count_dev, VM_ERR_BADARG, "NULL buffer");
    VM_REQUIRE(nq >= 1 && k >= 1 && k2 >= 1, VM_ERR_BADARG, "bad shape");
    DeviceGuard g(device);
    return k_merge_max_by_id(idx_dev, score_dev, count_dev, nq, k, k2, out_idx_dev, out_score_dev, out_count_dev,
                             (cudaStream_t)stream);
}

extern "C" int vm_cosine_pairs(int device, const void *a, const void *b, int dtype, int mem, int64_t n, int dim, int zero_rule,
                               int sum_mode, double *out, int out_mem, void *stream)
{
    VM_REQUIRE(n >= 0 && dim >= 0, VM_ERR_BADARG, "bad shape");
    VM_REQUIRE(dtype == VM_F32 || dtype == VM_F64, VM_ERR_BADARG, "dtype must be VM_F32 or VM_F64");
    VM_REQUIRE(zero_rule >= 0 && zero_rule <= 2, VM_ERR_BADARG, "zero_rule %d outside [0, 2]", zero_rule);
    if (n == 0) return VM_OK;
    VM_REQUIRE(a && b && out, VM_ERR_BADARG, "NULL buffer");
    int rc = check_arch(device, nullptr);
    if (rc != VM_OK) return rc;
    DeviceGuard g(device);
    cudaStream_t st = (cudaStream_t)stream;
    VM_REQUIRE(device >= 0 && device < MAX_DEVICES, VM_ERR_BADARG, "device index %d outside [0, %d)", device, MAX_DEVICES);
    static thread_local Buf scratch[MAX_DEVICES][3];
    Buf &da = scratch[device][0], &db = scratch[device][1], &dout = scratch[device][2];
    size_t bytes = (size_t)n * dim * dtype_size(dtype);
    const void *pa = a, *pb = b;
    if (mem == VM_MEM_HOST) {
        if ((rc = da.ensure(bytes ? bytes : 8)) != VM_OK || (rc = db.ensure(bytes ? bytes : 8)) != VM_OK) return rc;
        VM_CUDA_CHECK(cudaMemcpyAsync(da.p, a, bytes, cudaMemcpyHostToDevice, st));
        VM_CUDA_CHECK(cudaMemcpyAsync(db.p, b, bytes, cudaMemcpyHostToDevice, st));
        pa = da.p; pb = db.p;
    }
    double *po = out;
    if (out_mem == VM_MEM_HOST) {
        if ((rc = dout.ensure((size_t)n * 8)) != VM_OK) return rc;
        po = (double *)dout.p;
    }
    rc = k_cosine_pairs(pa, pb, dtype, n, dim, zero_rule, sum_mode, po, st);
    if (rc != VM_OK) return rc;
    if (out_mem == VM_MEM_HOST) {
        VM_CUDA_CHECK(cudaMemcpyAsync(out, po, (size_t)n * 8, cudaMemcpyDeviceToHost, st));
        VM_CUDA_CHECK(cudaStreamSynchronize(st));
    }
    return VM_OK;
}

extern "C" int vm_pairs_above(int device, const void *x_dev, int dtype, int64_t n, int dim, float threshold, int64_t cap,
                              int64_t *out_i_dev, int64_t *out_j_dev, float *out_score_dev, int64_t *out_count_dev, int part,
                              int nparts, int flags, void *stream)
{
    VM_REQUIRE(x_dev && out_count_dev, VM_ERR_BADARG, "NULL buffer");
    VM_REQUIRE(cap == 0 || (out_i_dev && out_j_dev && out_score_dev), VM_ERR_BADARG, "NULL output with cap > 0");
    VM_REQUIRE(dtype == VM_F32 || dtype == VM_BF16, VM_ERR_BADARG, "dtype must be VM_F32 or VM_BF16");
    VM_REQUIRE(n >= 0 && n < (1LL << 31), VM_ERR_BADARG, "n outside [0, 2^31)");
    VM_REQUIRE(dim >= 1 && dim <= 4096, VM_ERR_BADARG, "dim outside [1, 4096]");
    VM_REQUIRE(nparts >= 1 && part >= 0 && part < nparts, VM_ERR_BADARG, "bad part/nparts");
    int rc = check_arch(device, nullptr);
    if (rc != VM_OK) return rc;
    DeviceGuard g(device);
    return k_pairs_above(device, x_dev, dtype, n, dim, ld_for_dim(dim), threshold, cap, out_i_dev, out_j_dev, out_score_dev,
                         out_count_dev, part, nparts, flags, (cudaStream_t)stream);
}

extern "C" int vm_pairs_above_sharded(vm_comm *comm, void *x_dev, int dtype, int64_t n, int dim, float threshold, int64_t cap,
                                      int64_t *out_i_dev, int64_t *out_j_dev, float *out_score_dev, int64_t *out_count_dev,
                                      int root, int flags, void *stream)
{
    VM_REQUIRE(comm, VM_ERR_BADARG, "comm is NULL");
    VM_REQUIRE(x_dev && out_count_dev, VM_ERR_BADARG, "NULL buffer");
    VM_REQUIRE(cap >= 1 && out_i_dev && out_j_dev && out_score_dev, VM_ERR_BADARG, "cap < 1 or NULL output");
    VM_REQUIRE(dtype == VM_F32 || dtype == VM_BF16, VM_ERR_BADARG, "dtype must be VM_F32 or VM_BF16");
    VM_REQUIRE(n >= 0 && n < (1LL << 31), VM_ERR_BADARG, "n outside [0, 2^31)");
    VM_REQUIRE(dim >= 1 && dim <= 4096, VM_ERR_BADARG, "dim outside [1, 4096]");
    VM_REQUIRE(root >= -1 && root < comm->nranks, VM_ERR_BADARG, "root %d outside [-1, %d)", root, comm->nranks);
    int rc = check_arch(comm->device, nullptr);
    if (rc != VM_OK) return rc;
    DeviceGuard g(comm->device);
    cudaStream_t st = (cudaStream_t)stream;
    const int G = comm->nranks, ld = ld_for_dim(dim);
    if (root >= 0 && G > 1 && n > 0)
        VM_NCCL_CHECK(g_nccl.Broadcast(x_dev, x_dev, (size_t)n * ld * dtype_size(dtype),  0, root, comm->nccl, st));
#define ENS(b, bytes) if ((rc = (b).ensure(bytes)) != VM_OK) return rc
    ENS(comm->pl_i, (size_t)cap * 8); ENS(comm->pl_j, (size_t)cap * 8); ENS(comm->pl_s, (size_t)cap * 4);
    ENS(comm->pl_cnt, 8); ENS(comm->pg_cnt, (size_t)G * 8);
    if (!comm->h_counts) VM_CUDA_CHECK(cudaMallocHost((void **)&comm->h_counts, 16 * 8));
    rc = k_pairs_above(comm->device, x_dev, dtype, n, dim, ld, threshold, cap, (int64_t *)comm->pl_i.p, (int64_t *)comm->pl_j.p,
                       (float *)comm->pl_s.p, (int64_t *)comm->pl_cnt.p, comm->rank, G, 0, st);
    if (rc != VM_OK) return rc;
    VM_NCCL_CHECK(g_nccl.AllGather(comm->pl_cnt.p, comm->pg_cnt.p, 8,  0, comm->nccl, st));
    int64_t slot = cap;
    if (!(flags & VM_FLAG_ASYNC)) {
        VM_CUDA_CHECK(cudaMemcpyAsync(comm->h_counts, comm->pg_cnt.p, (size_t)G * 8, cudaMemcpyDeviceToHost, st));
        VM_CUDA_CHECK(cudaStreamSynchronize(st));
        int64_t mx = 0, total = 0;
        for (int r = 0; r < G; ++r) { mx = comm->h_counts[r] > mx ? comm->h_counts[r] : mx; total += comm->h_counts[r]; }
        if (mx > cap || total > cap) {
            VM_CUDA_CHECK(cudaMemcpyAsync(out_count_dev, &total, 8, cudaMemcpyHostToDevice, st));
            VM_CUDA_CHECK(cudaStreamSynchronize(st));
            set_error("%lld pairs above the threshold exceed cap=%lld", (long long)total, (long long)cap);
            return VM_ERR_OVERFLOW;
        }
        slot = mx;
    }
    if (slot == 0) { VM_CUDA_CHECK(cudaMemsetAsync(out_count_dev, 0, 8, st)); return VM_OK; }
    const size_t per_rank = ((size_t)slot * 20 + 7) & ~(size_t)7;
    ENS(comm->pg_send, per_rank); ENS(comm->pg_recv, per_rank * G);
#undef ENS
    char *sb = (char *)comm->pg_send.p;
    VM_CUDA_CHECK(cudaMemcpyAsync(sb, comm->pl_i.p, (size_t)slot * 8, cudaMemcpyDeviceToDevice, st));
    VM_CUDA_CHECK(cudaMemcpyAsync(sb + (size_t)slot * 8, comm->pl_j.p, (size_t)slot * 8, cudaMemcpyDeviceToDevice, st));
    VM_CUDA_CHECK(cudaMemcpyAsync(sb + (size_t)slot * 16, comm->pl_s.p, (size_t)slot * 4, cudaMemcpyDeviceToDevice, st));
    VM_NCCL_CHECK(g_nccl.AllGather(comm->pg_send.p, comm->pg_recv.p, per_rank,  0, comm->nccl, st));
    return k_pairs_concat(comm->pg_recv.p, per_rank, slot, (const int64_t *)comm->pg_cnt.p, G, cap, out_i_dev, out_j_dev,
                          out_score_dev, out_count_dev, st);
}

extern "C" int vm_comm_unique_id(void *out128)
{
    VM_REQUIRE(out128, VM_ERR_BADARG, "out is NULL");
    int rc = nccl_load();
    if (rc != VM_OK) return rc;
    VM_NCCL_CHECK(g_nccl.GetUniqueId(out128));
    return VM_OK;
}

extern "C" int vm_comm_init_rank(vm_comm **out, int device, int nranks, int rank, const void *id128)
{
    VM_REQUIRE(out && id128, VM_ERR_BADARG, "NULL argument");
    VM_REQUIRE(nranks >= 1 && nranks <= 16 && rank >= 0 && rank < nranks, VM_ERR_BADARG, "bad rank %d / nranks %d (at most 16 ranks)", rank, nranks);
    int rc = nccl_load();
    if (rc != VM_OK) return rc;
    DeviceGuard g(device);
    VM_CUDA_CHECK(cudaSetDevice(device));
    vm_comm *c = new (std::nothrow) vm_comm();
    VM_REQUIRE(c, VM_ERR_OOM, "host allocation failed");
    Id128 id;
    memcpy(id.b, id128, 128);
    int r = g_nccl.CommInitRank(&c->nccl, nranks, id, rank);
    if (r != 0) {
        set_error("ncclCommInitRank failed: %s", g_nccl.GetErrorString ? g_nccl.GetErrorString(r) : "?");
        delete c;
        return VM_ERR_NCCL;
    }
    c->nranks = nranks; c->rank = rank; c->device = device;
    *out = c;
    return VM_OK;
}

extern "C" size_t vm_comm_exchange_bytes(void) { return XCHG_BYTES; }

extern "C" int vm_comm_attach_peer_buffers(vm_comm *c, void *const *bufs, int nranks)
{
    VM_REQUIRE(c && bufs, VM_ERR_BADARG, "NULL argument");
    VM_REQUIRE(nranks == c->nranks && nranks <= 16, VM_ERR_BADARG, "peer buffers for %d ranks, communicator has %d (max 16)", nranks, c->nranks);
    for (int r = 0; r < nranks; ++r) {
        VM_REQUIRE(bufs[r] && ((uintptr_t)bufs[r] & 255) == 0, VM_ERR_BADARG, "peer buffer %d is NULL or not 256-byte aligned", r);
        c->peer[r] = bufs[r];
    }
    c->p2p = true;
    c->gen = 0;
    return VM_OK;
}

extern "C" int vm_comm_destroy(vm_comm *c)
{
    if (!c) return VM_OK;
    if (c->nccl && g_nccl.CommDestroy) g_nccl.CommDestroy(c->nccl);
    {
        DeviceGuard g(c->device);
        Buf *all[] = {&c->pl_i, &c->pl_j, &c->pl_s, &c->pl_cnt, &c->pg_cnt, &c->pg_send, &c->pg_recv};
        for (Buf *b : all) b->release();
        if (c->h_counts) cudaFreeHost(c->h_counts);
    }
    delete c;
    return VM_OK;
}
extern "C" int vm_comm_nranks(const vm_comm *c) { return c ? c->nranks : -1; }
extern "C" int vm_comm_rank(const vm_comm *c) { return c ? c->rank : -1; }

extern "C" int vm_synth_fill(int device, void *rows_dev, int dtype, uint64_t seed, int64_t row0, int64_t n, int dim,
                             uint64_t dup_period, void *stream)
{
    VM_REQUIRE(rows_dev, VM_ERR_BADARG, "rows is NULL");
    VM_REQUIRE(dtype == VM_F32 || dtype == VM_BF16, VM_ERR_BADARG, "dtype must be VM_F32 or VM_BF16");
    DeviceGuard g(device);
    return k_synth_fill(rows_dev, dtype, seed, row0, n, dim, ld_for_dim(dim), dup_period, (cudaStream_t)stream);
}
```

real-time-brain-inspired-video-memory_b200/csrc/pairs.cu:

```cuda
#include "tc_common.cuh"
#include "raster.h"
#include <stdlib.h>
#include <mutex>

namespace vm {
using namespace tc;

static constexpr int P_BM = 128, P_BN = 256;
static constexpr int P_STAGES = 4, P_ACC = 2, P_THREADS = 192;
static constexpr int P_A_BYTES = P_BM * 128, P_B_BYTES = P_BN * 128, P_STAGE_BYTES = P_A_BYTES + P_B_BYTES;
static constexpr int P_GJ_LOG2_SMALL = 3, P_GJ_LOG2_LARGE = 6;
#ifndef VM_PAIRS_HINT_A
#define VM_PAIRS_HINT_A L2_EVICT_NORMAL
#endif
#ifndef VM_PAIRS_HINT_B
#define VM_PAIRS_HINT_B L2_EVICT_NORMAL
#endif
static constexpr int64_t P_GJ_LARGE_FROM_ROWS = 1 << 18;

struct PairsParams {
    int64_t n;
    int nbi, nbj, KB;
    float thr, thr_lo;
    const float *inv;
    int32_t *st_i, *st_j;
    float *st_s;
    unsigned long long *st_cnt;
    long long st_cap;
    long long total_tiles;
    int part, nparts;
    int gj_log2;
    int groups;
    unsigned long long *prog;
};

template <bool TF32>
__global__ void __launch_bounds__(P_THREADS, 1)
pairs_tc_kernel(const __grid_constant__ CUtensorMap tmA, const __grid_constant__ CUtensorMap tmB, PairsParams p)
{
    extern __shared__ __align__(16) uint8_t smem_raw[];
    uint8_t *base = smem_raw + ((1024u - (smem_u32(smem_raw) & 1023u)) & 1023u);
    uint8_t *stages = base;
    float *sinv = reinterpret_cast<float *>(base + P_STAGES * P_STAGE_BYTES);
    uint64_t *bars = reinterpret_cast<uint64_t *>(sinv + P_ACC * P_BN);
    uint64_t *full = bars, *empty = bars + P_STAGES, *tfull = empty + P_STAGES, *tempty = tfull + P_ACC;
    uint32_t *tmem_slot = reinterpret_cast<uint32_t *>(tempty + P_ACC);

    const int warp = __shfl_sync(0xffffffffu, threadIdx.x >> 5, 0);
    const int lane = threadIdx.x & 31;
    constexpr int ELEMS = TF32 ? 32 : 64;

    if (warp == 0 && lane == 0) {
        tma_prefetch_desc(&tmA);
        tma_prefetch_desc(&tmB);
        for (int s = 0; s < P_STAGES; ++s) { mbar_init(&full[s], 1); mbar_init(&empty[s], 1); }
        for (int a = 0; a < P_ACC; ++a) { mbar_init(&tfull[a], 1); mbar_init(&tempty[a], 4); }
        fence_barrier_init();
    }
    if (warp == 1) tmem_alloc(tmem_slot, 512);
    tc_fence_before();
    __syncthreads();
    tc_fence_after();
    const uint32_t tmem_base = *tmem_slot;

    auto valid_tile = [&](int bi, int bj) {
        return bi < p.nbi && bj < p.nbj && ((long long)bj * P_BN + P_BN - 1 > (long long)bi * P_BM);
    };

    if (warp == 0) {
        if (lane == 0) {
            int stage = 0;
            uint32_t phase = 0;
            TileIter<2> ti;
            for (ti.init(blockIdx.x, gridDim.x, p.groups, p.gj_log2, p.part, p.nparts); ti.valid(); ti.next()) {
                const int bi = ti.bi(), bj = ti.bj();
                if (!valid_tile(bi, bj)) continue;
                for (int kb = 0; kb < p.KB; ++kb) {
                    mbar_wait(&empty[stage], phase ^ 1);
                    mbar_arrive_expect_tx(&full[stage], P_STAGE_BYTES);
                    uint8_t *sa = stages + (size_t)stage * P_STAGE_BYTES;
                    tma_load_2d(&tmA, &full[stage], sa, kb * ELEMS, bi * P_BM, L2_EVICT_FIRST);
                    tma_load_2d(&tmB, &full[stage], sa + P_A_BYTES, kb * ELEMS, bj * P_BN, L2_EVICT_LAST);
                    if (++stage == P_STAGES) { stage = 0; phase ^= 1; }
                }
            }
        }
    } else if (warp == 1) {
        if (lane == 0) {
            const uint32_t idesc = make_idesc(TF32 ? 2u : 1u, P_BM, P_BN);
            int stage = 0, acc = 0;
            uint32_t phase = 0, acc_phase = 0;
            const uint32_t s0 = smem_u32(stages);
            TileIter<2> ti;
            for (ti.init(blockIdx.x, gridDim.x, p.groups, p.gj_log2, p.part, p.nparts); ti.valid(); ti.next()) {
                const int bi = ti.bi(), bj = ti.bj();
                if (!valid_tile(bi, bj)) continue;
                mbar_wait(&tempty[acc], acc_phase ^ 1);
                tc_fence_after();
                const uint32_t d_tmem = tmem_base + (uint32_t)(acc * P_BN);
                for (int kb = 0; kb < p.KB; ++kb) {
                    mbar_wait(&full[stage], phase);
                    tc_fence_after();
                    const uint32_t a_addr = s0 + (uint32_t)stage * P_STAGE_BYTES;
                    const uint32_t b_addr = a_addr + P_A_BYTES;
#pragma unroll
                    for (int j = 0; j < 4; ++j)
                        umma<TF32>(d_tmem, make_smem_desc_sw128(a_addr + j * 32), make_smem_desc_sw128(b_addr + j * 32), idesc,
                                   (uint32_t)((kb | j) != 0));
                    umma_commit(&empty[stage]);
                    if (++stage == P_STAGES) { stage = 0; phase ^= 1; }
                }
                umma_commit(&tfull[acc]);
                if (++acc == P_ACC) { acc = 0; acc_phase ^= 1; }
            }
        }
    } else {
        const int e = threadIdx.x - 64;
        const int quad = warp & 3;
        const int row_in_tile = quad * 32 + lane;
        int acc = 0;
        uint32_t acc_phase = 0;
        TileIter<2> ti;
        for (ti.init(blockIdx.x, gridDim.x, p.groups, p.gj_log2, p.part, p.nparts); ti.valid(); ti.next()) {
            const int bi = ti.bi(), bj = ti.bj();
            if (!valid_tile(bi, bj)) continue;
            const long long i = (long long)bi * P_BM + row_in_tile;
            const long long j0 = (long long)bj * P_BN;
            const float inv_i = i < p.n ? __ldg(p.inv + i) : -1.0f;
            float *sj = sinv + acc * P_BN;
            for (int c = e; c < P_BN; c += 128) sj[c] = (j0 + c < p.n) ? __ldg(p.inv + j0 + c) : 0.0f;
            float thr_i;
            if (inv_i > 0.0f) thr_i = p.thr_lo / inv_i, thr_i -= fabsf(thr_i) * 1e-6f;
            else thr_i = (inv_i == 0.0f && 0.0f > p.thr_lo) ? -INFINITY : INFINITY;
            named_bar_sync(1, 128);
            mbar_wait(&tfull[acc], acc_phase);
            tc_fence_after();
            const uint32_t taddr = tmem_base + ((uint32_t)(quad * 32) << 16) + (uint32_t)(acc * P_BN);
#pragma unroll 1
            for (int c = 0; c < P_BN; c += 32) {
                uint32_t v[32];
                tmem_ld32(taddr + c, v);
                float w[32];
#pragma unroll
                for (int q4 = 0; q4 < 8; ++q4) {
                    const float4 t4 = *reinterpret_cast<const float4 *>(sj + c + 4 * q4);
                    w[4 * q4] = t4.x; w[4 * q4 + 1] = t4.y; w[4 * q4 + 2] = t4.z; w[4 * q4 + 3] = t4.w;
                }
                tmem_ld_wait();
                uint32_t hits = 0;
#pragma unroll
                for (int jj = 0; jj < 32; ++jj) hits |= (__uint_as_float(v[jj]) * w[jj] > thr_i) ? (1u << jj) : 0u;
                while (hits) {
                    const int jj = __ffs(hits) - 1;
                    hits &= hits - 1;
                    float a = 0.0f, wj = 0.0f;
#pragma unroll
                    for (int x = 0; x < 32; ++x) { a = (x == jj) ? __uint_as_float(v[x]) : a; wj = (x == jj) ? w[x] : wj; }
                    const long long j = j0 + c + jj;
                    const float s = a * wj * inv_i;
                    if (j < p.n && j > i && s > p.thr_lo) {
                        const unsigned long long pos = atomicAdd(p.st_cnt, 1ull);
                        if ((long long)pos < p.st_cap) { p.st_i[pos] = (int32_t)i; p.st_j[pos] = (int32_t)j; p.st_s[pos] = s; }
                    }
                }
            }
            tc_fence_before();
            __syncwarp();
            if (lane == 0) mbar_arrive(&tempty[acc]);
            if (++acc == P_ACC) { acc = 0; acc_phase ^= 1; }
        }
    }
    tc_fence_before();
    __syncthreads();
    if (warp == 1) {
        tc_fence_after();
        tmem_dealloc(tmem_base, 512);
    }
}

static constexpr int P2_STAGES = 6, P2_STAGE_BYTES = 2 * P_A_BYTES;

__device__ __forceinline__ void pairs_keep_pace(const unsigned long long *prog, long long my_step, long long window)
{
    if (my_step <= window) return;
    for (int spin = 0; spin < 64; ++spin) {
        unsigned long long done;
        asm volatile("ld.relaxed.gpu.global.u64 %0, [%1];" : "=l"(done) : "l"(prog) : "memory");
        if ((long long)done + window >= my_step) return;
        __nanosleep(256);
    }
}

template <bool TF32>
__global__ void __cluster_dims__(2, 1, 1) __launch_bounds__(P_THREADS, 1)
pairs_tc2_kernel(const __grid_constant__ CUtensorMap tmA, PairsParams p)
{
    extern __shared__ __align__(16) uint8_t smem_raw[];
    uint8_t *base = smem_raw + ((1024u - (smem_u32(smem_raw) & 1023u)) & 1023u);
    uint8_t *stages = base;
    float *sinv = reinterpret_cast<float *>(base + P2_STAGES * P2_STAGE_BYTES);
    uint64_t *bars = reinterpret_cast<uint64_t *>(sinv + P_ACC * P_BN);
    uint64_t *full = bars, *empty = bars + P2_STAGES, *tfull = empty + P2_STAGES, *tempty = tfull + P_ACC;
    uint32_t *tmem_slot = reinterpret_cast<uint32_t *>(tempty + P_ACC);

    const int warp = __shfl_sync(0xffffffffu, threadIdx.x >> 5, 0);
    const int lane = threadIdx.x & 31;
    const uint32_t rank = cluster_ctarank();
    const int pair = blockIdx.x >> 1, npairs = gridDim.x >> 1;
    constexpr int ELEMS = TF32 ? 32 : 64;

    if (warp == 0 && lane == 0) {
        tma_prefetch_desc(&tmA);
        for (int s = 0; s < P2_STAGES; ++s) { mbar_init(&full[s], 1); mbar_init(&empty[s], 1); }
        for (int a = 0; a < P_ACC; ++a) { mbar_init(&tfull[a], 1); mbar_init(&tempty[a], 8); }
        fence_barrier_init();
    }
    if (warp == 1) tmem_alloc_2sm(tmem_slot, 512);
    tc_fence_before();
    cluster_sync_all();
    tc_fence_after();
    const uint32_t tmem_base = *tmem_slot;
    const int nb = (int)((p.n + 255) / 256);

    auto valid_tile = [&](int bi, int bj) { return bi < nb && bj < nb && bj >= bi; };

    if (warp == 0) {
        if (lane == 0) {
            int stage = 0;
            uint32_t phase = 0;
            TileIter<1> ti;
            long long step = 0;
            const long long window = 4ll * npairs;
            for (ti.init(pair, npairs, p.groups, p.gj_log2, p.part, p.nparts); ti.valid(); ti.next(), ++step) {
                const int bi = ti.bi(), bj = ti.bj();
                if (!valid_tile(bi, bj)) continue;
                if (rank == 0) pairs_keep_pace(p.prog, step * npairs, window);
                for (int kb = 0; kb < p.KB; ++kb) {
                    mbar_wait(&empty[stage], phase ^ 1);
                    if (rank == 0) mbar_arrive_expect_tx(&full[stage], 2 * P2_STAGE_BYTES);
                    uint8_t *sa = stages + (size_t)stage * P2_STAGE_BYTES;
                    tma_load_2d_2sm(&tmA, &full[stage], sa, kb * ELEMS, bi * 256 + (int)rank * 128, VM_PAIRS_HINT_A);
                    tma_load_2d_2sm(&tmA, &full[stage], sa + P_A_BYTES, kb * ELEMS, bj * 256 + (int)rank * 128, VM_PAIRS_HINT_B);
                    if (++stage == P2_STAGES) { stage = 0; phase ^= 1; }
                }
            }
        }
    } else if (warp == 1) {
        if (lane == 0 && rank == 0) {
            const uint32_t idesc = make_idesc(TF32 ? 2u : 1u, 256, 256);
            int stage = 0, acc = 0;
            uint32_t phase = 0, acc_phase = 0;
            const uint32_t s0 = smem_u32(stages);
            TileIter<1> ti;
            for (ti.init(pair, npairs, p.groups, p.gj_log2, p.part, p.nparts); ti.valid(); ti.next()) {
                const int bi = ti.bi(), bj = ti.bj();
                atomicAdd(p.prog, 1ull);
                if (!valid_tile(bi, bj)) continue;
                mbar_wait(&tempty[acc], acc_phase ^ 1);
                tc_fence_after();
                const uint32_t d_tmem = tmem_base + (uint32_t)(acc * P_BN);
                for (int kb = 0; kb < p.KB; ++kb) {
                    mbar_wait(&full[stage], phase);
                    tc_fence_after();
                    const uint32_t a_addr = s0 + (uint32_t)stage * P2_STAGE_BYTES;
                    const uint32_t b_addr = a_addr + P_A_BYTES;
#pragma unroll
                    for (int j = 0; j < 4; ++j)
                        umma_2sm<TF32>(d_tmem, make_smem_desc_sw128(a_addr + j * 32), make_smem_desc_sw128(b_addr + j * 32), idesc,
                                       (uint32_t)((kb | j) != 0));
                    umma_commit_2sm(&empty[stage]);
                    if (++stage == P2_STAGES) { stage = 0; phase ^= 1; }
                }
                umma_commit_2sm(&tfull[acc]);
                if (++acc == P_ACC) { acc = 0; acc_phase ^= 1; }
            }
        }
    } else {
        const int e = threadIdx.x - 64;
        const int quad = warp & 3;
        const int row_in_tile = quad * 32 + lane;
        int acc = 0;
        uint32_t acc_phase = 0;
        TileIter<1> ti;
        for (ti.init(pair, npairs, p.groups, p.gj_log2, p.part, p.nparts); ti.valid(); ti.next()) {
            const int bi = ti.bi(), bj = ti.bj();
            if (!valid_tile(bi, bj)) continue;
            const long long i = (long long)bi * 256 + rank * 128 + row_in_tile;
            const long long j0 = (long long)bj * 256;
            const float inv_i = i < p.n ? __ldg(p.inv + i) : -1.0f;
            float *sj = sinv + acc * P_BN;
            for (int c = e; c < P_BN; c += 128) sj[c] = (j0 + c < p.n) ? __ldg(p.inv + j0 + c) : 0.0f;
            float thr_i;
            if (inv_i > 0.0f) thr_i = p.thr_lo / inv_i, thr_i -= fabsf(thr_i) * 1e-6f;
            else thr_i = (inv_i == 0.0f && 0.0f > p.thr_lo) ? -INFINITY : INFINITY;
            named_bar_sync(1, 128);
            mbar_wait(&tfull[acc], acc_phase);
            tc_fence_after();
            const uint32_t taddr = tmem_base + ((uint32_t)(quad * 32) << 16) + (uint32_t)(acc * P_BN);
#pragma unroll 1
            for (int c = 0; c < P_BN; c += 32) {
                uint32_t v[32];
                tmem_ld32(taddr + c, v);
                float w[32];
#pragma unroll
                for (int q4 = 0; q4 < 8; ++q4) {
                    const float4 t4 = *reinterpret_cast<const float4 *>(sj + c + 4 * q4);
                    w[4 * q4] = t4.x; w[4 * q4 + 1] = t4.y; w[4 * q4 + 2] = t4.z; w[4 * q4 + 3] = t4.w;
                }
                tmem_ld_wait();
                uint32_t hits = 0;
#pragma unroll
                for (int jj = 0; jj < 32; ++jj) hits |= (__uint_as_float(v[jj]) * w[jj] > thr_i) ? (1u << jj) : 0u;
                while (hits) {
                    const int jj = __ffs(hits) - 1;
                    hits &= hits - 1;
                    float a = 0.0f, wj = 0.0f;
#pragma unroll
                    for (int x = 0; x < 32; ++x) { a = (x == jj) ? __uint_as_float(v[x]) : a; wj = (x == jj) ? w[x] : wj; }
                    const long long j = j0 + c + jj;
                    const float s = a * wj * inv_i;
                    if (j < p.n && j > i && s > p.thr_lo) {
                        const unsigned long long pos = atomicAdd(p.st_cnt, 1ull);
                        if ((long long)pos < p.st_cap) { p.st_i[pos] = (int32_t)i; p.st_j[pos] = (int32_t)j; p.st_s[pos] = s; }
                    }
                }
            }
            tc_fence_before();
            __syncwarp();
            if (lane == 0) {
                if (rank == 0) mbar_arrive(&tempty[acc]);
                else mbar_arrive_remote(&tempty[acc], 0);
            }
            if (++acc == P_ACC) { acc = 0; acc_phase ^= 1; }
        }
    }
    tc_fence_before();
    cluster_sync_all();
    if (warp == 1) {
        tc_fence_after();
        tmem_dealloc_2sm(tmem_base, 512);
    }
}

template <typename T>
__global__ void pairs_finalize_kernel(const T *__restrict__ x, int ld, int dim, float thr, float eps,
                                      const int32_t *__restrict__ st_i, const int32_t *__restrict__ st_j,
                                      const float *__restrict__ st_s, const unsigned long long *__restrict__ st_cnt,
                                      long long st_cap, int64_t *__restrict__ out_i, int64_t *__restrict__ out_j,
                                      float *__restrict__ out_s, unsigned long long *__restrict__ out_cnt, long long cap)
{
    const unsigned long long staged = *st_cnt;
    const long long m = (long long)(staged < (unsigned long long)st_cap ? staged : (unsigned long long)st_cap);
    for (long long e = blockIdx.x * (long long)blockDim.x + threadIdx.x; e < m; e += (long long)gridDim.x * blockDim.x) {
        const int i = st_i[e], j = st_j[e];
        float s = st_s[e];
        bool keep = s > thr;
        if (fabsf(s - thr) <= eps) {
            const T *a = x + (int64_t)i * ld, *b = x + (int64_t)j * ld;
            double dot = 0.0, aa = 0.0, bb = 0.0;
            for (int c = 0; c < dim; ++c) {
                const double u = (double)load_as_float(a, c), v = (double)load_as_float(b, c);
                dot += u * v; aa += u * u; bb += v * v;
            }
            const double den = sqrt(aa) * sqrt(bb);
            const double ex = den > 0.0 ? dot / den : 0.0;
            keep = ex > (double)thr;
            s = (float)ex;
        }
        if (keep) {
            const unsigned long long pos = atomicAdd(out_cnt, 1ull);
            if ((long long)pos < cap) { out_i[pos] = i; out_j[pos] = j; out_s[pos] = s; }
        }
    }
    if (blockIdx.x == 0 && threadIdx.x == 0 && staged > (unsigned long long)st_cap) atomicMax(out_cnt, staged);
}

__global__ void pairs_concat_kernel(const char *__restrict__ gathered, size_t per_rank_bytes, long long slot,
                                    const long long *__restrict__ counts, int nranks, long long cap, int64_t *__restrict__ out_i,
                                    int64_t *__restrict__ out_j, float *__restrict__ out_s, long long *__restrict__ out_count)
{
    const int r = blockIdx.y;
    long long off = 0, total = 0;
    for (int q = 0; q < nranks; ++q) { if (q < r) off += counts[q]; total += counts[q]; }
    const long long m = counts[r] < slot ? counts[r] : slot;
    const char *b = gathered + (size_t)r * per_rank_bytes;
    const int64_t *gi = reinterpret_cast<const int64_t *>(b), *gj = reinterpret_cast<const int64_t *>(b + (size_t)slot * 8);
    const float *gs = reinterpret_cast<const float *>(b + (size_t)slot * 16);
    for (long long e = blockIdx.x * (long long)blockDim.x + threadIdx.x; e < m; e += (long long)gridDim.x * blockDim.x)
        if (off + e < cap) { out_i[off + e] = gi[e]; out_j[off + e] = gj[e]; out_s[off + e] = gs[e]; }
    if (r == 0 && blockIdx.x == 0 && threadIdx.x == 0) *out_count = total;
}

int k_pairs_concat(const void *gathered, size_t per_rank_bytes, int64_t slot, const int64_t *counts, int nranks, int64_t cap,
                   int64_t *out_i, int64_t *out_j, float *out_score, int64_t *out_count, cudaStream_t st)
{
    dim3 grid((unsigned)imin64((slot + 255) / 256, 256), (unsigned)nranks);
    pairs_concat_kernel<<<grid, 256, 0, st>>>((const char *)gathered, per_rank_bytes, (long long)slot, (const long long *)counts, nranks,
                                             (long long)cap, out_i, out_j, out_score, (long long *)out_count);
    VM_CUDA_CHECK(cudaGetLastError());
    return VM_OK;
}

int k_row_inv_norms(const void *rows, int dtype, float *inv_norms, int64_t row0, int64_t n, int ld, int *extreme, cudaStream_t st,
                    const double *exact = nullptr);

namespace {
struct PairsWs {
    void *inv = nullptr, *st_i = nullptr, *st_j = nullptr, *st_s = nullptr, *cnt = nullptr;
    size_t inv_bytes = 0, st_entries = 0;
    cudaStream_t stream = nullptr;
    bool used = false;
};
constexpr int PWS_STREAMS = 8;
PairsWs g_pws[16][PWS_STREAMS];
std::mutex g_pws_mu;
PairsWs *pairs_ws(int device, cudaStream_t st)
{
    std::lock_guard<std::mutex> lock(g_pws_mu);
    PairsWs *free_slot = nullptr;
    for (PairsWs &w : g_pws[device]) {
        if (w.used && w.stream == st) return &w;
        if (!w.used && !free_slot) free_slot = &w;
    }
    if (free_slot) { free_slot->used = true; free_slot->stream = st; }
    return free_slot;
}
int ensure(void **p, size_t *have, size_t need)
{
    if (need <= *have) return VM_OK;
    if (*p) cudaFree(*p);
    *p = nullptr; *have = 0;
    cudaError_t e = cudaMalloc(p, need);
    if (e != cudaSuccess) { set_error("cudaMalloc(%zu) failed: %s", need, cudaGetErrorString(e)); return VM_ERR_OOM; }
    *have = need;
    return VM_OK;
}
}

int k_pairs_above(int device, const void *x, int dtype, int64_t n, int dim, int ld, float threshold, int64_t cap,
                  int64_t *out_i, int64_t *out_j, float *out_score, int64_t *out_count, int part, int nparts, int flags,
                  cudaStream_t st)
{
    (void)flags;
    VM_REQUIRE(device >= 0 && device < 16, VM_ERR_BADARG, "device index %d outside [0, 16)", device);
    VM_CUDA_CHECK(cudaMemsetAsync(out_count, 0, 8, st));
    if (n <= 1) return VM_OK;
    VM_REQUIRE(((uintptr_t)x & 127) == 0, VM_ERR_BADARG, "rows buffer must be 128-byte aligned");
    PairsWs *wp = pairs_ws(device, st);
    VM_REQUIRE(wp, VM_ERR_UNSUPPORTED, "all-pairs scorer: more than %d distinct streams in use on device %d", PWS_STREAMS, device);
    PairsWs &w = *wp;
    int rc = ensure(&w.inv, &w.inv_bytes, (size_t)n * 4);
    if (rc != VM_OK) return rc;
    const size_t st_cap = (size_t)cap + ((size_t)cap / 8 > 65536 ? (size_t)cap / 8 : 65536);
    if (st_cap > w.st_entries) {
        size_t have;
        have = w.st_entries * 4; rc = ensure(&w.st_i, &have, st_cap * 4); if (rc != VM_OK) return rc;
        have = w.st_entries * 4; rc = ensure(&w.st_j, &have, st_cap * 4); if (rc != VM_OK) return rc;
        have = w.st_entries * 4; rc = ensure(&w.st_s, &have, st_cap * 4); if (rc != VM_OK) return rc;
        w.st_entries = st_cap;
    }
    if (!w.cnt) VM_CUDA_CHECK(cudaMalloc(&w.cnt, 16));
    VM_CUDA_CHECK(cudaMemsetAsync(w.cnt, 0, 16, st));
    rc = k_row_inv_norms(x, dtype, (float *)w.inv, 0, n, ld, nullptr, st);
    if (rc != VM_OK) return rc;

    const int es = dtype == VM_F32 ? 4 : 2;
    const float fp32_acc = (float)(dim + 32) * 1.1920928955078125e-07f;
    const float eps = dtype == VM_F32 ? 3.90625e-3f + fp32_acc : fp32_acc;
    PairsParams p{};
    p.n = n;
    p.nbi = (int)((n + P_BM - 1) / P_BM);
    p.nbj = (int)((n + P_BN - 1) / P_BN);
    p.KB = (ld * es + 127) / 128;
    p.thr = threshold;
    p.thr_lo = threshold - eps;
    p.inv = (const float *)w.inv;
    p.st_i = (int32_t *)w.st_i; p.st_j = (int32_t *)w.st_j; p.st_s = (float *)w.st_s;
    p.st_cnt = (unsigned long long *)w.cnt;
    p.prog = (unsigned long long *)w.cnt + 1;
    p.st_cap = (long long)st_cap;
    p.gj_log2 = n >= P_GJ_LARGE_FROM_ROWS ? P_GJ_LOG2_LARGE : P_GJ_LOG2_SMALL;
    const long long P_GJ = 1ll << p.gj_log2;
    const long long groups = (p.nbj + P_GJ - 1) / P_GJ;
    p.groups = (int)groups;
    p.total_tiles = P_GJ * P_GJ * groups * (groups + 1);
    p.part = part; p.nparts = nparts;

    CUtensorMap tmA, tmB;
    rc = make_tmap_2d(&tmA, x, dtype, (uint64_t)n, (uint64_t)ld, (uint64_t)ld, P_BM);
    if (rc != VM_OK) return rc;
    int sms = 148;
    cudaDeviceGetAttribute(&sms, cudaDevAttrMultiProcessorCount, device);
#ifdef VIDMEM_TRIAGE_KERNELS
    static const bool one_cta = getenv("VIDMEM_PAIRS_1CTA") != nullptr;
#else
    constexpr bool one_cta = false;
#endif
    if (!one_cta) {
        const long long nb = (n + 255) / 256, groups = (nb + P_GJ - 1) / P_GJ;
        p.total_tiles = P_GJ * P_GJ * groups * (groups + 1) / 2;
        const size_t smem = (size_t)P2_STAGES * P2_STAGE_BYTES + P_ACC * P_BN * 4 + 8 * (2 * P2_STAGES + 2 * P_ACC) + 16 + 1024;
        const long long my_tiles = (p.total_tiles + nparts - 1) / nparts;
        long long pairs = sms / 2;
        if (my_tiles < pairs) pairs = my_tiles;
        const int grid = (int)(2 * pairs);
        if (dtype == VM_F32) {
            VM_CUDA_CHECK((max_smem_once<pairs_tc2_kernel<true>>(227 * 1024)));
            pairs_tc2_kernel<true><<<grid, P_THREADS, smem, st>>>(tmA, p);
        } else {
            VM_CUDA_CHECK((max_smem_once<pairs_tc2_kernel<false>>(227 * 1024)));
            pairs_tc2_kernel<false><<<grid, P_THREADS, smem, st>>>(tmA, p);
        }
    } else {
        rc = make_tmap_2d(&tmB, x, dtype, (uint64_t)n, (uint64_t)ld, (uint64_t)ld, P_BN);
        if (rc != VM_OK) return rc;
        const size_t smem = (size_t)P_STAGES * P_STAGE_BYTES + P_ACC * P_BN * 4 + 8 * (2 * P_STAGES + 2 * P_ACC) + 16 + 1024;
        const long long my_tiles = (p.total_tiles + nparts - 1) / nparts;
        const int grid = (int)(my_tiles < sms ? my_tiles : sms);
        if (dtype == VM_F32) {
            VM_CUDA_CHECK((max_smem_once<pairs_tc_kernel<true>>(227 * 1024)));
            pairs_tc_kernel<true><<<grid, P_THREADS, smem, st>>>(tmA, tmB, p);
        } else {
            VM_CUDA_CHECK((max_smem_once<pairs_tc_kernel<false>>(227 * 1024)));
            pairs_tc_kernel<false><<<grid, P_THREADS, smem, st>>>(tmA, tmB, p);
        }
    }
    VM_CUDA_CHECK(cudaGetLastError());
    if (dtype == VM_F32)
        pairs_finalize_kernel<float><<<64, 256, 0, st>>>((const float *)x, ld, dim, threshold, eps, p.st_i, p.st_j, p.st_s, p.st_cnt,
                                                         p.st_cap, out_i, out_j, out_score, (unsigned long long *)out_count, cap);
    else
        pairs_finalize_kernel<__nv_bfloat16><<<64, 256, 0, st>>>((const __nv_bfloat16 *)x, ld, dim, threshold, eps, p.st_i, p.st_j,
                                                                 p.st_s, p.st_cnt, p.st_cap, out_i, out_j, out_score,
                                                                 (unsigned long long *)out_count, cap);
    VM_CUDA_CHECK(cudaGetLastError());
    return VM_OK;
}

}
```

real-time-brain-inspired-video-memory_b200/csrc/store.cu:

```cuda
#include "common.cuh"
#include "synth.cuh"

namespace vm {

template <typename DST>
__global__ void convert_rows_kernel(const void *__restrict__ src, int src_dtype, DST *__restrict__ dst, int64_t n,
                                    int dim, int ld)
{
    int64_t total = n * (int64_t)ld;
    for (int64_t e = blockIdx.x * (int64_t)blockDim.x + threadIdx.x; e < total; e += (int64_t)gridDim.x * blockDim.x) {
        int64_t r = e / ld;
        int c = (int)(e - r * ld);
        double dv = 0.0;
        if (c < dim) dv = load_as_double(src, src_dtype, r * dim + c);
        if constexpr (sizeof(DST) == 8) dst[e] = dv;
        else {
            const float v = (float)dv;
            if constexpr (sizeof(DST) == 4) dst[e] = v;
            else dst[e] = __float2bfloat16_rn(v);
        }
    }
}

template <typename T>
__global__ void row_inv_norms_kernel(const T *__restrict__ rows, float *__restrict__ inv_norms, int64_t row0,
                                     int64_t n, int ld, int *__restrict__ extreme, const double *__restrict__ exact)
{
    int lane = threadIdx.x & 31;
    int64_t warp = (blockIdx.x * (int64_t)blockDim.x + threadIdx.x) >> 5;
    int64_t nwarps = ((int64_t)gridDim.x * blockDim.x) >> 5;
    for (int64_t r = row0 + warp; r < n; r += nwarps) {
        const T *p = rows + r * (int64_t)ld;
        double ss = 0.0;
        for (int c = lane; c < ld; c += 32) {
            double v = (double)load_as_float(p, c);
            ss += v * v;
        }
        for (int o = 16; o > 0; o >>= 1) ss += __shfl_xor_sync(0xffffffffu, ss, o);
        double se = 0.0;
        if (exact != nullptr) {
            for (int c = lane; c < ld; c += 32) {
                const double v = exact[r * (int64_t)ld + c] * 0x1p-600;
                se += v * v;
            }
            for (int o = 16; o > 0; o >>= 1) se += __shfl_xor_sync(0xffffffffu, se, o);
        }
        if (lane == 0) {
            float inv = 0.0f;
            if (!isfinite(ss)) {
                inv = -1.0f;
                if (exact != nullptr && isfinite(se)) { inv = 0.0f; if (extreme) atomicAdd(extreme, 1); }
            } else if (ss > 0.0) {
                inv = (float)(1.0 / sqrt(ss));
                if (extreme && (ss < 7.52316384526264e-37 || ss > 1.329227995784916e+36)) atomicAdd(extreme, 1);
            } else if (exact != nullptr && se != 0.0) {
                if (extreme) atomicAdd(extreme, 1);
            }
            inv_norms[r] = inv;
        }
    }
}

__global__ void invalidate_rows_kernel(float *inv_norms, const int64_t *rows, int64_t n, int64_t size)
{
    int64_t i = blockIdx.x * (int64_t)blockDim.x + threadIdx.x;
    if (i < n && rows[i] >= 0 && rows[i] < size) inv_norms[rows[i]] = -1.0f;
}

__global__ void normalize_queries_kernel(const void *__restrict__ q, int q_dtype, int nq, int nq_pad, int dim, int ld,
                                         float *__restrict__ out_f32, __nv_bfloat16 *__restrict__ out_bf16,
                                         int32_t *__restrict__ zero_me, uint32_t *__restrict__ zero_tab, int zero_tab_n,
                                         int tf32_round, int split)
{
    pdl_launch_dependents();
    pdl_wait();
    if (zero_me && blockIdx.x == 0 && threadIdx.x < 2) zero_me[threadIdx.x] = 0;
    for (int i = blockIdx.x * blockDim.x + threadIdx.x; i < zero_tab_n; i += gridDim.x * blockDim.x) zero_tab[i] = 0u;
    int lane = threadIdx.x & 31;
    int w = (blockIdx.x * blockDim.x + threadIdx.x) >> 5;
    if (w >= nq_pad) return;
    double ss = 0.0;
    if (w < nq)
        for (int c = lane; c < dim; c += 32) {
            double v = load_as_double(q, q_dtype, (int64_t)w * dim + c);
            ss += v * v;
        }
    for (int o = 16; o > 0; o >>= 1) ss += __shfl_xor_sync(0xffffffffu, ss, o);
    double inv = (ss > 0.0 && isfinite(ss)) ? 1.0 / sqrt(ss) : 0.0;
    for (int c = lane; c < ld; c += 32) {
        float v = 0.0f;
        if (w < nq && c < dim) v = (float)(load_as_double(q, q_dtype, (int64_t)w * dim + c) * inv);
        float vf = v;
        if (tf32_round) vf = __uint_as_float((__float_as_uint(v) + 0x1000u) & 0xFFFFE000u);
        out_f32[(int64_t)w * ld + c] = vf;
        if (out_bf16) {
            const __nv_bfloat16 hi = __float2bfloat16_rn(v);
            out_bf16[(int64_t)w * ld + c] = hi;
            if (split) out_bf16[((int64_t)nq_pad + w) * ld + c] = __float2bfloat16_rn(v - __bfloat162float(hi));
        }
    }
}

template <typename T>
__global__ void synth_fill_kernel(T *__restrict__ rows, uint64_t seed, int64_t row0, int64_t n, int dim, int ld,
                                  uint64_t dup_period)
{
    int groups = ld >> 3;
    int64_t total = n * (int64_t)groups;
    uint64_t hk = splitmix64(seed ^ 0xD6E8FEB86659FD93ULL);
    for (int64_t e = blockIdx.x * (int64_t)blockDim.x + threadIdx.x; e < total; e += (int64_t)gridDim.x * blockDim.x) {
        int64_t i = e / groups;
        int g = (int)(e - i * groups);
        uint64_t row = (uint64_t)(row0 + i);
        uint64_t own = splitmix64(splitmix64(seed * 0x9E3779B97F4A7C15ULL + row) + (uint64_t)g);
        uint64_t par = 0, sel = 0;
        bool planted = false;
        if (dup_period > 0 && row > 0) {
            uint64_t hr = splitmix64(hk + row);
            if (hr % dup_period == 0) {
                planted = true;
                uint64_t parent = splitmix64(hr) % row;
                par = splitmix64(splitmix64(seed * 0x9E3779B97F4A7C15ULL + parent) + (uint64_t)g);
                sel = splitmix64(hr + 0x632BE59BD9B4E019ULL + (uint64_t)g);
            }
        }
        T *dst = rows + i * (int64_t)ld + g * 8;
#pragma unroll
        for (int b = 0; b < 8; ++b) {
            int col = g * 8 + b;
            int v = synth_int(own, b);
            if (planted && (((sel >> (8 * b)) & 15ULL) != 0ULL)) v = synth_int(par, b);
            float f = col < dim ? (float)v * (1.0f / 128.0f) : 0.0f;
            if constexpr (sizeof(T) == 4) dst[b] = f;
            else dst[b] = __float2bfloat16_rn(f);
        }
    }
}

int k_convert_rows(const void *src, int src_dtype, void *dst, int dst_dtype, int64_t n, int dim, int ld, cudaStream_t st)
{
    if (n <= 0) return VM_OK;
    int64_t total = n * (int64_t)ld;
    int grid = (int)vm::imin64((total + 255) / 256, 148 * 16);
    if (dst_dtype == VM_F32) convert_rows_kernel<float><<<grid, 256, 0, st>>>(src, src_dtype, (float *)dst, n, dim, ld);
    else if (dst_dtype == VM_F64) convert_rows_kernel<double><<<grid, 256, 0, st>>>(src, src_dtype, (double *)dst, n, dim, ld);
    else convert_rows_kernel<__nv_bfloat16><<<grid, 256, 0, st>>>(src, src_dtype, (__nv_bfloat16 *)dst, n, dim, ld);
    VM_CUDA_CHECK(cudaGetLastError());
    return VM_OK;
}

int k_row_inv_norms(const void *rows, int dtype, float *inv_norms, int64_t row0, int64_t n, int ld, int *extreme, cudaStream_t st,
                    const double *exact)
{
    if (n <= row0) return VM_OK;
    int64_t warps = n - row0;
    int grid = (int)vm::imin64((warps * 32 + 255) / 256, 148 * 16);
    if (dtype == VM_F32) row_inv_norms_kernel<float><<<grid, 256, 0, st>>>((const float *)rows, inv_norms, row0, n, ld, extreme, exact);
    else row_inv_norms_kernel<__nv_bfloat16><<<grid, 256, 0, st>>>((const __nv_bfloat16 *)rows, inv_norms, row0, n, ld, extreme, exact);
    VM_CUDA_CHECK(cudaGetLastError());
    return VM_OK;
}

int k_invalidate_rows(float *inv_norms, const int64_t *rows_dev, int64_t n, int64_t size, cudaStream_t st)
{
    if (n <= 0) return VM_OK;
    invalidate_rows_kernel<<<(int)((n + 255) / 256), 256, 0, st>>>(inv_norms, rows_dev, n, size);
    VM_CUDA_CHECK(cudaGetLastError());
    return VM_OK;
}

int k_normalize_queries(const void *q, int q_dtype, int nq, int nq_pad, int dim, int ld, float *out_f32,
                        void *out_bf16, int32_t *zero_me, uint32_t *zero_tab, int zero_tab_n, int tf32_round, int split, bool pdl,
                        cudaStream_t st)
{
    int threads = 128;
    int grid = (nq_pad * 32 + threads - 1) / threads;
    VM_CUDA_CHECK(launch_pdl(normalize_queries_kernel, dim3(grid), dim3(threads), 0, st, pdl, q, q_dtype, nq, nq_pad, dim, ld, out_f32,
                             (__nv_bfloat16 *)out_bf16, zero_me, zero_tab, zero_tab_n, tf32_round, split));
    VM_CUDA_CHECK(cudaGetLastError());
    return VM_OK;
}

int k_synth_fill(void *rows, int dtype, uint64_t seed, int64_t row0, int64_t n, int dim, int ld, uint64_t dup_period,
                 cudaStream_t st)
{
    if (n <= 0) return VM_OK;
    int64_t total = n * (int64_t)(ld >> 3);
    int grid = (int)vm::imin64((total + 255) / 256, 148 * 32);
    if (dtype == VM_F32) synth_fill_kernel<float><<<grid, 256, 0, st>>>((float *)rows, seed, row0, n, dim, ld, dup_period);
    else synth_fill_kernel<__nv_bfloat16><<<grid, 256, 0, st>>>((__nv_bfloat16 *)rows, seed, row0, n, dim, ld, dup_period);
    VM_CUDA_CHECK(cudaGetLastError());
    return VM_OK;
}

}
```

real-time-brain-inspired-video-memory_b200/store.py:

```python
from __future__ import annotations

import ctypes as C
import math
from typing import Iterable, List, Optional, Sequence, Tuple

import numpy as np
import torch

from . import _lib as L

_DT = {"f32": L.VM_F32, "fp32": L.VM_F32, "float32": L.VM_F32, "bf16": L.VM_BF16, "bfloat16": L.VM_BF16}
_DT_EXACT = {"f64": L.VM_F32, "fp64": L.VM_F32, "float64": L.VM_F32, "f64+f32": L.VM_F32, "f64+bf16": L.VM_BF16}
_TORCH_DT = {L.VM_F32: torch.float32, L.VM_BF16: torch.bfloat16}


def _np_dtype_code(a: np.ndarray) -> int:
    if a.dtype == np.float32:
        return L.VM_F32
    if a.dtype == np.float64:
        return L.VM_F64
    raise TypeError(f"unsupported host dtype {a.dtype}")


def _torch_dtype_code(t: torch.Tensor) -> int:
    if t.dtype == torch.float32:
        return L.VM_F32
    if t.dtype == torch.bfloat16:
        return L.VM_BF16
    if t.dtype == torch.float64:
        return L.VM_F64
    raise TypeError(f"unsupported tensor dtype {t.dtype}")


_raw_stream = getattr(torch._C, "_cuda_getCurrentRawStream", None)


def _stream_ptr(device: torch.device) -> int:
    if _raw_stream is not None:
        return _raw_stream(device.index)
    return torch.cuda.current_stream(device).cuda_stream


def device_row_limit(dim: int, dtype: str, device: int = 0) -> int:
    per_row = ((int(dim) + 7) & ~7) * {"f32": 4, "bf16": 2, "f64+bf16": 10}.get(dtype, 12) + 4
    total = torch.cuda.get_device_properties(device).total_memory if torch.cuda.is_available() else 1 << 34
    return max(1, min(total // per_row, (1 << 31) - 512))


class _DeviceRange:

    def __init__(self, ptr: int, shape, typestr: str):
        self.__cuda_array_interface__ = {"shape": tuple(shape), "typestr": typestr, "data": (int(ptr), False),
                                         "version": 3, "strides": None}


class EmbeddingStore:

    def __init__(self, dim: int, capacity: int, dtype: str = "f32", device: int = 0, _buffers=None,
                 max_capacity: Optional[int] = None):
        if not torch.cuda.is_available():
            raise RuntimeError("EmbeddingStore needs a CUDA device (sm_100); there is no CPU fallback")
        self.lib = L.load()
        self.dim, self.capacity = int(dim), int(capacity)
        self.growable = max_capacity is not None
        self.dtype = str(dtype)
        self.exact = dtype in _DT_EXACT
        self.dtype_code = _DT_EXACT[dtype] if self.exact else _DT[dtype]
        self.device = torch.device("cuda", device)
        self.ld = self.lib.vm_ld(self.dim)
        self.rows_exact = None
        if self.growable:
            h = C.c_void_p()
            with torch.cuda.device(self.device):
                L.check(self.lib.vm_store_create_growable(C.byref(h), device, self.dim, self.dtype_code, 1 if self.exact else 0,
                                                          self.capacity, max(int(max_capacity), self.capacity)))
            self._h = h
            self.max_capacity = int(self.lib.vm_store_max_capacity(h))
            self._refresh_views()
            self.last_stats = L.TopkStats()
            self._stats_ref = C.byref(self.last_stats)
            return
        self.max_capacity = self.capacity
        if _buffers is None:
            self.rows = torch.empty((self.capacity, self.ld), dtype=_TORCH_DT[self.dtype_code], device=self.device)
            self.inv_norms = torch.empty((self.capacity,), dtype=torch.float32, device=self.device)
            if self.exact:
                self.rows_exact = torch.empty((self.capacity, self.ld), dtype=torch.float64, device=self.device)
        elif self.exact:
            self.rows, self.inv_norms, self.rows_exact = _buffers
        else:
            self.rows, self.inv_norms = _buffers
        h = C.c_void_p()
        if self.exact:
            L.check(self.lib.vm_store_attach_exact(C.byref(h), device, self.dim, self.dtype_code, self.capacity,
                                                   self.rows.data_ptr(), self.inv_norms.data_ptr(), self.rows_exact.data_ptr()))
        else:
            L.check(self.lib.vm_store_attach(C.byref(h), device, self.dim, self.dtype_code, self.capacity,
                                             self.rows.data_ptr(), self.inv_norms.data_ptr()))
        self._h = h
        self.last_stats = L.TopkStats()
        self._stats_ref = C.byref(self.last_stats)

    def _refresh_views(self) -> None:
        self.capacity = cap = int(self.lib.vm_store_capacity(self._h))
        dev = self.device
        if self.dtype_code == L.VM_BF16:
            r = torch.as_tensor(_DeviceRange(self.lib.vm_store_rows_ptr(self._h), (cap, self.ld), "<i2"), device=dev).view(torch.bfloat16)
        else:
            r = torch.as_tensor(_DeviceRange(self.lib.vm_store_rows_ptr(self._h), (cap, self.ld), "<f4"), device=dev)
        self.rows = r
        self.inv_norms = torch.as_tensor(_DeviceRange(self.lib.vm_store_inv_norms_ptr(self._h), (cap,), "<f4"), device=dev)
        if self.exact:
            self.rows_exact = torch.as_tensor(_DeviceRange(self.lib.vm_store_rows_exact_ptr(self._h), (cap, self.ld), "<f8"), device=dev)

    def reserve(self, capacity: int) -> None:
        if int(capacity) <= self.capacity:
            return
        if not self.growable:
            raise ValueError(f"store over fixed buffers of {self.capacity} rows cannot grow; create it with max_capacity")
        L.check(self.lib.vm_store_reserve(self._h, int(capacity)))
        self._refresh_views()

    def resident_bytes(self) -> int:
        return int(self.lib.vm_store_resident_bytes(self._h))

    def prefix_view(self, n: int) -> "EmbeddingStore":
        n = int(n)
        if not 1 <= n <= len(self):
            raise ValueError(f"prefix of {n} rows outside [1, {len(self)}]")
        bufs = (self.rows[:n], self.inv_norms[:n]) + ((self.rows_exact[:n],) if self.exact else ())
        v = EmbeddingStore(self.dim, n, self.dtype, self.device.index, _buffers=bufs)
        L.check(self.lib.vm_store_set_size(v._h, n, n, _stream_ptr(self.device)))
        return v

    def close(self) -> None:
        if getattr(self, "_h", None):
            if self.growable:
                self.rows = self.inv_norms = self.rows_exact = None
            self.lib.vm_store_destroy(self._h)
            self._h = None

    def __del__(self):
        try:
            self.close()
        except Exception:
            pass

    def __len__(self) -> int:
        return int(self.lib.vm_store_size(self._h))

    def _src(self, rows) -> Tuple[int, int, int, int, object]:
        if isinstance(rows, torch.Tensor):
            t = rows.contiguous()
            if t.dim() != 2 or t.shape[1] != self.dim:
                raise ValueError(f"expected [n, {self.dim}] rows, got {tuple(t.shape)}")
            if t.is_cuda:
                return t.data_ptr(), _torch_dtype_code(t), L.VM_MEM_DEVICE, t.shape[0], t
            if t.dtype == torch.bfloat16:
                return t.data_ptr(), L.VM_BF16, L.VM_MEM_HOST, t.shape[0], t
            rows = t.numpy()
        a = np.asarray(rows)
        if a.dtype not in (np.float32, np.float64):
            a = a.astype(np.float64)
        a = np.ascontiguousarray(a)
        if a.ndim != 2 or a.shape[1] != self.dim:
            raise ValueError(f"expected [n, {self.dim}] rows, got {a.shape}")
        return a.ctypes.data, _np_dtype_code(a), L.VM_MEM_HOST, a.shape[0], a

    def append(self, rows) -> int:
        ptr, dt, mem, n, keep = self._src(rows)
        first = C.c_int64(-1)
        L.check(self.lib.vm_store_append(self._h, ptr, dt, mem, n, C.byref(first), _stream_ptr(self.device)))
        if self.growable and int(first.value) + n > self.capacity:
            self._refresh_views()
        if mem == L.VM_MEM_HOST:
            torch.cuda.current_stream(self.device).synchronize()
        return int(first.value)

    def update(self, row0: int, rows) -> None:
        ptr, dt, mem, n, keep = self._src(rows)
        L.check(self.lib.vm_store_update(self._h, int(row0), ptr, dt, mem, n, _stream_ptr(self.device)))
        if mem == L.VM_MEM_HOST:
            torch.cuda.current_stream(self.device).synchronize()

    def invalidate(self, rows: Sequence[int]) -> None:
        a = np.ascontiguousarray(np.asarray(list(rows), dtype=np.int64))
        L.check(self.lib.vm_store_invalidate(self._h, a.ctypes.data, a.size, _stream_ptr(self.device)))
        torch.cuda.current_stream(self.device).synchronize()

    def set_size(self, n: int, recompute_from_row: int = 0) -> None:
        L.check(self.lib.vm_store_set_size(self._h, int(n), int(recompute_from_row), _stream_ptr(self.device)))

    def last_scan_ms(self) -> float:
        ms = C.c_float(0.0)
        L.check(self.lib.vm_store_last_scan_ms(self._h, C.byref(ms)))
        return float(ms.value)

    def avg_scan_ms(self):
        ms, n = C.c_float(0.0), C.c_int(0)
        L.check(self.lib.vm_store_avg_scan_ms(self._h, C.byref(ms), C.byref(n)))
        return float(ms.value), int(n.value)

    def counters(self, reset: bool = False) -> dict:
        c = L.StoreCounters()
        L.check(self.lib.vm_store_read_counters(self._h, C.byref(c), 1 if reset else 0))
        return c.as_dict()

    def band_keys(self):
        kept, spilled, n = (C.c_int64 * 64)(), (C.c_int64 * 64)(), C.c_int(0)
        L.check(self.lib.vm_store_band_keys(self._h, 64, kept, spilled, C.byref(n)))
        return np.array(kept[:n.value], np.int64), np.array(spilled[:n.value], np.int64)

    def clear(self) -> None:
        L.check(self.lib.vm_store_clear(self._h))

    def synth_fill(self, seed: int, n: int, row0: int = 0, dup_period: int = 0, first_buffer_row: int = 0) -> None:
        dst = self.rows[first_buffer_row:first_buffer_row + n]
        L.check(self.lib.vm_synth_fill(self.device.index, dst.data_ptr(), self.dtype_code, seed, row0, n, self.dim,
                                       dup_period, _stream_ptr(self.device)))

    def save(self, path: str, ids: Optional[Sequence[str]] = None, extra: Optional[dict] = None) -> None:
        n = len(self)
        if self.exact:
            raw = self.rows_exact[:n, :self.dim].contiguous().cpu().numpy()
        else:
            rows = self.rows[:n, :self.dim].contiguous()
            raw = rows.view(torch.int16).cpu().numpy().view(np.uint16) if self.dtype_code == L.VM_BF16 else rows.cpu().numpy()
        skipped = (self.inv_norms[:n] < 0).cpu().numpy()
        arrays = {"rows": raw, "skipped": skipped, "dim": np.int64(self.dim), "dtype": np.int64(self.dtype_code),
                  "exact": np.int64(1 if self.exact else 0),
                  "ids": np.asarray([str(x) for x in ids] if ids is not None else [], dtype=np.str_)}
        for name, text in (extra or {}).items():
            arrays["extra_" + name] = np.frombuffer(str(text).encode("utf-8"), dtype=np.uint8)
        np.savez(path, **arrays)

    @classmethod
    def load(cls, path: str, capacity: Optional[int] = None, device: int = 0, with_extra: bool = False,
             min_capacity: int = 1, max_capacity: Optional[int] = None):
        z = np.load(path if path.endswith(".npz") else path + ".npz", allow_pickle=False)
        dim, code = int(z["dim"]), int(z["dtype"])
        raw = z["rows"]
        n = raw.shape[0]
        exact = "exact" in z.files and int(z["exact"]) == 1
        name = ("f64+bf16" if code == L.VM_BF16 else "f64") if exact else ("bf16" if code == L.VM_BF16 else "f32")
        if max_capacity == "auto":
            max_capacity = device_row_limit(dim, name, device)
        cap = max(int(capacity or n), int(min_capacity), 1)
        st = cls(dim, cap, name, device, max_capacity=None if max_capacity is None else max(int(max_capacity), cap))
        if n:
            if code == L.VM_BF16 and not exact:
                t = torch.from_numpy(raw.view(np.int16).copy()).view(torch.bfloat16)
                st.append(t.to(st.device))
            else:
                st.append(raw)
            bad = np.nonzero(z["skipped"])[0]
            if len(bad):
                st.invalidate(bad)
        ids = [str(x) for x in z["ids"].tolist()]
        if not with_extra:
            return st, ids
        extra = {k[len("extra_"):]: bytes(z[k].tobytes()).decode("utf-8") for k in z.files if k.startswith("extra_")}
        return st, ids, extra

    def topk(self, queries, k: int, min_score: float = -math.inf, score_mode: int = L.VM_SCORE_RAW,
             sum_mode: Optional[int] = None, flags: int = 0, comm=None, row_offset: int = 0):
        if isinstance(queries, torch.Tensor) and queries.is_cuda:
            raise TypeError("use topk_device for CUDA tensors")
        q = np.asarray(queries.numpy() if isinstance(queries, torch.Tensor) else queries)
        if q.dtype not in (np.float32, np.float64):
            q = q.astype(np.float64)
        q = np.ascontiguousarray(q)
        if q.ndim != 2 or q.shape[1] != self.dim:
            raise ValueError(f"expected [nq, {self.dim}] queries, got {q.shape}")
        nq = q.shape[0]
        idx = np.full((nq, k), -1, np.int64)
        score = np.zeros((nq, k), np.float64)
        count = np.zeros((nq,), np.int32)
        sm = L.DEFAULT_SUM_MODE if sum_mode is None else sum_mode
        st = _stream_ptr(self.device)
        if comm is None:
            rc = self.lib.vm_topk(self._h, q.ctypes.data, _np_dtype_code(q), L.VM_MEM_HOST, nq, k, float(min_score),
                                  score_mode, sm, flags, idx.ctypes.data, score.ctypes.data, count.ctypes.data,
                                  L.VM_MEM_HOST, self._stats_ref, st)
        else:
            rc = self.lib.vm_topk_sharded(self._h, comm.handle, int(row_offset), q.ctypes.data, _np_dtype_code(q),
                                          L.VM_MEM_HOST, nq, k, float(min_score), score_mode, sm, flags,
                                          idx.ctypes.data, score.ctypes.data, count.ctypes.data, L.VM_MEM_HOST,
                                          self._stats_ref, st)
        L.check(rc)
        return idx, score, count

    def topk_device(self, queries: torch.Tensor, k: int, out=None, min_score: float = -math.inf,
                    score_mode: int = L.VM_SCORE_RAW, sum_mode: Optional[int] = None, flags: int = 0, comm=None,
                    row_offset: int = 0):
        if not queries.is_cuda:
            raise TypeError("queries must be a CUDA tensor")
        if queries.device != self.device:
            raise ValueError(f"queries live on {queries.device}, the store on {self.device}")
        if queries.dim() != 2 or queries.shape[1] != self.dim:
            raise ValueError(f"expected [nq, {self.dim}] queries, got {tuple(queries.shape)}")
        if not 1 <= int(k) <= 64:
            raise ValueError(f"k = {k} outside [1, 64]")
        q = queries.contiguous()
        nq = q.shape[0]
        if out is not None:
            want = ((nq, k), torch.int64), ((nq, k), torch.float64), ((nq,), torch.int32)
            if len(out) != 3:
                raise ValueError("out must be (idx, score, count)")
            for t, (shape, dt) in zip(out, want):
                if (not isinstance(t, torch.Tensor) or t.device != self.device or t.dtype != dt
                        or tuple(t.shape) != shape or not t.is_contiguous()):
                    raise ValueError(f"out tensors must be contiguous {want} on {self.device}")
        if out is None:
            out = (torch.empty((nq, k), dtype=torch.int64, device=self.device),
                   torch.empty((nq, k), dtype=torch.float64, device=self.device),
                   torch.empty((nq,), dtype=torch.int32, device=self.device))
        idx, score, count = out
        sm = L.DEFAULT_SUM_MODE if sum_mode is None else sum_mode
        st = _stream_ptr(self.device)
        if comm is None:
            rc = self.lib.vm_topk(self._h, q.data_ptr(), _torch_dtype_code(q), L.VM_MEM_DEVICE, nq, k, float(min_score),
                                  score_mode, sm, flags, idx.data_ptr(), score.data_ptr(), count.data_ptr(),
                                  L.VM_MEM_DEVICE, self._stats_ref, st)
        else:
            rc = self.lib.vm_topk_sharded(self._h, comm.handle, int(row_offset), q.data_ptr(), _torch_dtype_code(q),
                                          L.VM_MEM_DEVICE, nq, k, float(min_score), score_mode, sm, flags,
                                          idx.data_ptr(), score.data_ptr(), count.data_ptr(), L.VM_MEM_DEVICE,
                                          self._stats_ref, st)
        L.check(rc)
        return idx, score, count


def cosine_pairs(a, b, zero_rule: int = 0, sum_mode: Optional[int] = None, device: int = 0) -> np.ndarray:
    lib = L.load()
    a = np.ascontiguousarray(np.asarray(a, dtype=np.float64))
    b = np.ascontiguousarray(np.asarray(b, dtype=np.float64))
    if a.ndim == 1:
        a, b = a[None, :], b[None, :]
    if a.shape != b.shape:
        raise ValueError("shape mismatch")
    out = np.zeros(a.shape[0], np.float64)
    sm = L.DEFAULT_SUM_MODE if sum_mode is None else sum_mode
    dev = torch.device("cuda", device)
    L.check(lib.vm_cosine_pairs(device, a.ctypes.data, b.ctypes.data, L.VM_F64, L.VM_MEM_HOST, a.shape[0], a.shape[1],
                                zero_rule, sm, out.ctypes.data, L.VM_MEM_HOST, _stream_ptr(dev)))
    return out
```

Measured before the change: 260,000.

## Scan f32 stores through a bf16 shadow copy and rescore against exact f32 rows

F32 stores now keep a bf16 shadow copy of every row, refreshed on append, update and resize. The tensor-core scan reads the shadow, which halves the bytes streamed per row. Candidates are then rescored against the original f32 rows, and the certification epsilon is widened to cover bf16 rounding. The costs are extra memory per row, a conversion on every write, and possibly more uncertified candidates or rescans because the error band is wider.

```diff
diff --git a/include/vidmem.h b/include/vidmem.h
--- a/include/vidmem.h
+++ b/include/vidmem.h
@@ -59,6 +59,8 @@
 int vm_store_create(vm_store **out, int device, int dim, int dtype, int64_t capacity);
 int vm_store_attach(vm_store **out, int device, int dim, int dtype, int64_t capacity, void *rows_dev,
                     float *inv_norms_dev);
+int vm_store_attach_shadow(vm_store **out, int device, int dim, int64_t capacity, float *rows_dev, float *inv_norms_dev,
+                           void *shadow_dev);
 int vm_store_create_exact(vm_store **out, int device, int dim, int shadow_dtype, int64_t capacity);
 int vm_store_attach_exact(vm_store **out, int device, int dim, int shadow_dtype, int64_t capacity, void *rows_dev,
                           float *inv_norms_dev, double *rows_exact_dev);
@@ -70,6 +72,7 @@
 void *vm_store_rows_ptr(const vm_store *s);
 float *vm_store_inv_norms_ptr(const vm_store *s);
 double *vm_store_rows_exact_ptr(const vm_store *s);
+void *vm_store_shadow_ptr(const vm_store *s);
 int vm_store_destroy(vm_store *s);
 int64_t vm_store_size(const vm_store *s);
 int64_t vm_store_capacity(const vm_store *s);
diff --git a/real-time-brain-inspired-video-memory_b200/_lib.py b/real-time-brain-inspired-video-memory_b200/_lib.py
--- a/real-time-brain-inspired-video-memory_b200/_lib.py
+++ b/real-time-brain-inspired-video-memory_b200/_lib.py
@@ -19,8 +19,8 @@
 
 EXPORTS = [
     "vm_version", "vm_last_error", "vm_device_info", "vm_ld",
-    "vm_store_create", "vm_store_attach", "vm_store_create_exact", "vm_store_attach_exact", "vm_store_create_growable", "vm_store_reserve",
-    "vm_store_max_capacity", "vm_store_resident_bytes", "vm_store_rows_ptr", "vm_store_inv_norms_ptr", "vm_store_rows_exact_ptr", "vm_store_destroy", "vm_store_size", "vm_store_capacity", "vm_store_dim",
+    "vm_store_create", "vm_store_attach", "vm_store_create_exact", "vm_store_attach_exact", "vm_store_attach_shadow", "vm_store_create_growable", "vm_store_reserve",
+    "vm_store_max_capacity", "vm_store_resident_bytes", "vm_store_rows_ptr", "vm_store_inv_norms_ptr", "vm_store_rows_exact_ptr", "vm_store_shadow_ptr", "vm_store_destroy", "vm_store_size", "vm_store_capacity", "vm_store_dim",
     "vm_store_ld", "vm_store_append", "vm_store_update", "vm_store_invalidate", "vm_store_set_size", "vm_store_clear",
     "vm_store_last_scan_ms",
     "vm_store_avg_scan_ms", "vm_store_read_counters", "vm_store_band_keys",
@@ -74,6 +74,7 @@
         "vm_store_attach": (ci, [P(vp), ci, ci, ci, i64, vp, vp]),
         "vm_store_create_exact": (ci, [P(vp), ci, ci, ci, i64]),
         "vm_store_attach_exact": (ci, [P(vp), ci, ci, ci, i64, vp, vp, vp]),
+        "vm_store_attach_shadow": (ci, [P(vp), ci, ci, i64, vp, vp, vp]),
         "vm_store_create_growable": (ci, [P(vp), ci, ci, ci, ci, i64, i64]),
         "vm_store_reserve": (ci, [vp, i64]),
         "vm_store_max_capacity": (i64, [vp]),
@@ -81,6 +82,7 @@
         "vm_store_rows_ptr": (vp, [vp]),
         "vm_store_inv_norms_ptr": (vp, [vp]),
         "vm_store_rows_exact_ptr": (vp, [vp]),
+        "vm_store_shadow_ptr": (vp, [vp]),
         "vm_store_destroy": (ci, [vp]),
         "vm_store_size": (i64, [vp]),
         "vm_store_capacity": (i64, [vp]),
diff --git a/real-time-brain-inspired-video-memory_b200/csrc/api.cu b/real-time-brain-inspired-video-memory_b200/csrc/api.cu
--- a/real-time-brain-inspired-video-memory_b200/csrc/api.cu
+++ b/real-time-brain-inspired-video-memory_b200/csrc/api.cu
@@ -21,7 +21,7 @@
 
 int k_convert_rows(const void *src, int src_dtype, void *dst, int dst_dtype, int64_t n, int dim, int ld, cudaStream_t st);
 int k_row_inv_norms(const void *rows, int dtype, float *inv_norms, int64_t row0, int64_t n, int ld, int *extreme, cudaStream_t st,
-                    const double *exact = nullptr);
+                    const void *exact = nullptr, int exact_dtype = VM_F64);
 int k_invalidate_rows(float *inv_norms, const int64_t *rows_dev, int64_t n, int64_t size, cudaStream_t st);
 int k_normalize_queries(const void *q, int q_dtype, int nq, int nq_pad, int dim, int ld, float *out_f32, void *out_bf16,
                         int32_t *zero_me, uint32_t *zero_tab, int zero_tab_n, int tf32_round, int split, bool pdl, cudaStream_t st);
@@ -143,11 +143,16 @@
     void *rows = nullptr;
     float *inv_norms = nullptr;
     double *rows_exact = nullptr;
+    void *shadow = nullptr;
     bool owns = false;
-    Arena *ar_rows = nullptr, *ar_inv = nullptr, *ar_exact = nullptr;
+    Arena *ar_rows = nullptr, *ar_inv = nullptr, *ar_exact = nullptr, *ar_shadow = nullptr;
     int64_t max_capacity = 0;
     const void *exact_rows() const { return rows_exact ? (const void *)rows_exact : (const void *)rows; }
     int exact_dtype() const { return rows_exact ? (int)VM_F64 : dtype; }
+    const void *scan_rows() const { return shadow ? shadow : rows; }
+    int scan_dtype() const { return shadow ? (int)VM_BF16 : dtype; }
+    bool scan_shadowed() const { return scan_rows() != exact_rows(); }
+    size_t row_bytes() const { return (size_t)ld * (dtype_size(dtype) + (rows_exact ? 8 : 0) + (shadow ? 2 : 0)) + 4; }
     int *extreme = nullptr;
     unsigned long long *cum = nullptr;
     int64_t n_batches = 0, n_queries = 0;
@@ -277,11 +282,11 @@
 }
 
 static double scan_eps_stored(int kernel, int store_dtype, int dim, int split);
-static double scan_eps(int kernel, int store_dtype, int dim, int split, bool shadow = false)
-{
-    const double base = scan_eps_stored(kernel, store_dtype, dim, split);
+static double scan_eps(int kernel, int scan_dtype, int dim, int split, bool shadow = false)
+{
+    const double base = scan_eps_stored(kernel, scan_dtype, dim, split);
     if (!shadow) return base;
-    return base + (store_dtype == VM_F32 ? 1.1920928955078125e-07 : 1.953125e-3 * 1.01);
+    return base + (scan_dtype == VM_F32 ? 1.1920928955078125e-07 : 3.90625e-3 * 1.01);
 }
 static double scan_eps_stored(int kernel, int store_dtype, int dim, int split)
 {
@@ -335,18 +340,21 @@
     return VM_OK;
 }
 
-extern "C" int vm_store_create(vm_store **out, int device, int dim, int dtype, int64_t capacity)
+static int store_create(vm_store **out, int device, int dim, int dtype, int64_t capacity, bool exact)
 {
     int rc = store_new(out, device, dim, dtype, capacity);
     if (rc != VM_OK) return rc;
     vm_store *s = *out;
     DeviceGuard g(device);
     s->owns = true;
-    size_t bytes = (size_t)capacity * s->ld * dtype_size(dtype);
-    cudaError_t e = cudaMalloc(&s->rows, bytes);
+    const size_t cells = (size_t)capacity * s->ld;
+    cudaError_t e = cudaMalloc(&s->rows, cells * dtype_size(dtype));
     if (e == cudaSuccess) e = cudaMalloc((void **)&s->inv_norms, (size_t)capacity * 4);
+    if (e == cudaSuccess && exact) e = cudaMalloc((void **)&s->rows_exact, cells * 8);
+    else if (e == cudaSuccess && dtype == VM_F32) e = cudaMalloc(&s->shadow, cells * 2);
     if (e != cudaSuccess) {
-        set_error("store allocation of %zu bytes failed: %s", bytes, cudaGetErrorString(e));
+        set_error("store allocation of %lld rows (%zu bytes per row) failed: %s", (long long)capacity,
+                  (size_t)s->ld * (dtype_size(dtype) + (exact ? 8 : dtype == VM_F32 ? 2 : 0)) + 4, cudaGetErrorString(e));
         vm_store_destroy(s);
         *out = nullptr;
         return VM_ERR_OOM;
@@ -354,21 +362,14 @@
     return VM_OK;
 }
 
+extern "C" int vm_store_create(vm_store **out, int device, int dim, int dtype, int64_t capacity)
+{
+    return store_create(out, device, dim, dtype, capacity, false);
+}
+
 extern "C" int vm_store_create_exact(vm_store **out, int device, int dim, int shadow_dtype, int64_t capacity)
 {
-    int rc = vm_store_create(out, device, dim, shadow_dtype, capacity);
-    if (rc != VM_OK) return rc;
-    vm_store *s = *out;
-    DeviceGuard g(device);
-    const size_t bytes = (size_t)capacity * s->ld * 8;
-    cudaError_t e = cudaMalloc((void **)&s->rows_exact, bytes);
-    if (e != cudaSuccess) {
-        set_error("store allocation of %zu bytes (binary64 rows) failed: %s", bytes, cudaGetErrorString(e));
-        vm_store_destroy(s);
-        *out = nullptr;
-        return VM_ERR_OOM;
-    }
-    return VM_OK;
+    return store_create(out, device, dim, shadow_dtype, capacity, true);
 }
 
 static int store_back(vm_store *s, int64_t capacity)
@@ -376,6 +377,7 @@
     int rc = arena_grow(s->ar_rows, (size_t)capacity * s->ld * dtype_size(s->dtype));
     if (rc == VM_OK) rc = arena_grow(s->ar_inv, (size_t)capacity * 4);
     if (rc == VM_OK && s->ar_exact) rc = arena_grow(s->ar_exact, (size_t)capacity * s->ld * 8);
+    if (rc == VM_OK && s->ar_shadow) rc = arena_grow(s->ar_shadow, (size_t)capacity * s->ld * 2);
     return rc;
 }
 
@@ -392,11 +394,13 @@
     rc = arena_create(&s->ar_rows, device, (size_t)max_capacity * s->ld * dtype_size(dtype));
     if (rc == VM_OK) rc = arena_create(&s->ar_inv, device, (size_t)max_capacity * 4);
     if (rc == VM_OK && exact) rc = arena_create(&s->ar_exact, device, (size_t)max_capacity * s->ld * 8);
+    else if (rc == VM_OK && dtype == VM_F32) rc = arena_create(&s->ar_shadow, device, (size_t)max_capacity * s->ld * 2);
     if (rc == VM_OK) rc = store_back(s, initial_capacity);
     if (rc != VM_OK) { vm_store_destroy(s); *out = nullptr; return rc; }
     s->rows = arena_base(s->ar_rows);
     s->inv_norms = (float *)arena_base(s->ar_inv);
     if (exact) s->rows_exact = (double *)arena_base(s->ar_exact);
+    if (s->ar_shadow) s->shadow = arena_base(s->ar_shadow);
     return VM_OK;
 }
 
@@ -418,11 +422,24 @@
 extern "C" void *vm_store_rows_ptr(const vm_store *s) { return s ? s->rows : nullptr; }
 extern "C" float *vm_store_inv_norms_ptr(const vm_store *s) { return s ? s->inv_norms : nullptr; }
 extern "C" double *vm_store_rows_exact_ptr(const vm_store *s) { return s ? s->rows_exact : nullptr; }
+extern "C" void *vm_store_shadow_ptr(const vm_store *s) { return s ? s->shadow : nullptr; }
 extern "C" size_t vm_store_resident_bytes(const vm_store *s)
 {
     if (!s) return 0;
-    if (s->ar_rows) return arena_mapped(s->ar_rows) + arena_mapped(s->ar_inv) + (s->ar_exact ? arena_mapped(s->ar_exact) : 0);
-    return (size_t)s->capacity * ((size_t)s->ld * (dtype_size(s->dtype) + (s->rows_exact ? 8 : 0)) + 4);
+    if (s->ar_rows)
+        return arena_mapped(s->ar_rows) + arena_mapped(s->ar_inv) + (s->ar_exact ? arena_mapped(s->ar_exact) : 0) +
+               (s->ar_shadow ? arena_mapped(s->ar_shadow) : 0);
+    return (size_t)s->capacity * s->row_bytes();
+}
+
+extern "C" int vm_store_attach_shadow(vm_store **out, int device, int dim, int64_t capacity, float *rows_dev, float *inv_norms_dev,
+                                      void *shadow_dev)
+{
+    VM_REQUIRE(shadow_dev && ((uintptr_t)shadow_dev & 127) == 0, VM_ERR_BADARG, "bf16 shadow buffer must be 128-byte aligned");
+    int rc = vm_store_attach(out, device, dim, VM_F32, capacity, rows_dev, inv_norms_dev);
+    if (rc != VM_OK) return rc;
+    (*out)->shadow = shadow_dev;
+    return VM_OK;
 }
 
 extern "C" int vm_store_attach_exact(vm_store **out, int device, int dim, int shadow_dtype, int64_t capacity, void *rows_dev,
@@ -453,8 +470,8 @@
     if (!s) return VM_OK;
     DeviceGuard g(s->device);
     cudaDeviceSynchronize();
-    if (s->owns) { cudaFree(s->rows); cudaFree(s->inv_norms); if (s->rows_exact) cudaFree(s->rows_exact); }
-    arena_destroy(s->ar_rows); arena_destroy(s->ar_inv); arena_destroy(s->ar_exact);
+    if (s->owns) { cudaFree(s->rows); cudaFree(s->inv_norms); if (s->rows_exact) cudaFree(s->rows_exact); if (s->shadow) cudaFree(s->shadow); }
+    arena_destroy(s->ar_rows); arena_destroy(s->ar_inv); arena_destroy(s->ar_exact); arena_destroy(s->ar_shadow);
     if (s->extreme) cudaFree(s->extreme);
     if (s->cum) cudaFree(s->cum);
     s->stage.release(); s->stage_idx.release();
@@ -470,6 +487,18 @@
 extern "C" int64_t vm_store_capacity(const vm_store *s) { return s ? s->capacity : -1; }
 extern "C" int vm_store_dim(const vm_store *s) { return s ? s->dim : -1; }
 extern "C" int vm_store_ld(const vm_store *s) { return s ? s->ld : -1; }
+
+static int store_derive(vm_store *s, int64_t r0, int64_t n, cudaStream_t st)
+{
+    if (n <= r0) return VM_OK;
+    if (s->shadow) {
+        const int rc = k_convert_rows((const float *)s->rows + (size_t)r0 * s->ld, VM_F32, (char *)s->shadow + (size_t)r0 * s->ld * 2,
+                                      VM_BF16, n - r0, s->ld, s->ld, st);
+        if (rc != VM_OK) return rc;
+    }
+    return k_row_inv_norms(s->scan_rows(), s->scan_dtype(), s->inv_norms, r0, n, s->ld, s->extreme, st,
+                           s->scan_shadowed() ? s->exact_rows() : nullptr, s->exact_dtype());
+}
 
 static int store_write(vm_store *s, int64_t row0, const void *rows, int src_dtype, int src_mem, int64_t n, cudaStream_t st)
 {
@@ -492,7 +521,7 @@
         rc = k_convert_rows(src, src_dtype, s->rows_exact + (size_t)row0 * s->ld, VM_F64, n, s->dim, s->ld, st);
         if (rc != VM_OK) return rc;
     }
-    return k_row_inv_norms(s->rows, s->dtype, s->inv_norms, row0, row0 + n, s->ld, s->extreme, st, s->rows_exact);
+    return store_derive(s, row0, row0 + n, st);
 }
 
 extern "C" int vm_store_append(vm_store *s, const void *rows, int src_dtype, int src_mem, int64_t n, int64_t *first_row,
@@ -501,8 +530,7 @@
     VM_REQUIRE(s, VM_ERR_BADARG, "store is NULL");
     VM_REQUIRE(n >= 0, VM_ERR_BADARG, "n < 0");
     if (s->ar_rows && s->size + n > s->capacity) {
-        const int64_t row_bytes = (int64_t)s->ld * (int64_t)(dtype_size(s->dtype) + (s->rows_exact ? 8 : 0)) + 4;
-        const int64_t slack_rows = ((int64_t)256 << 20) / row_bytes + 1;
+        const int64_t slack_rows = ((int64_t)256 << 20) / (int64_t)s->row_bytes() + 1;
         int64_t want = s->size + n + slack_rows;
         if (want > s->max_capacity) want = s->max_capacity;
         if (want >= s->size + n) {
@@ -557,7 +585,7 @@
                                     s->rows_exact + (size_t)r0 * s->ld, VM_F64, n - r0, s->ld, s->ld, (cudaStream_t)stream);
             if (rc != VM_OK) return rc;
         }
-        return k_row_inv_norms(s->rows, s->dtype, s->inv_norms, recompute_from_row, n, s->ld, s->extreme, (cudaStream_t)stream, s->rows_exact);
+        return store_derive(s, recompute_from_row, n, (cudaStream_t)stream);
     }
     return VM_OK;
 }
@@ -662,7 +690,7 @@
     static const bool block = [] { const char *e = getenv("VIDMEM_SYNC"); return e && !strcmp(e, "block"); }();
     if (block) return cudaStreamSynchronize(st);
     if (s) {
-        const double est_us = (double)s->size * s->ld * (double)dtype_size(s->dtype) / 6.5e6;
+        const double est_us = (double)s->size * s->ld * (double)dtype_size(s->scan_dtype()) / 6.5e6;
         if (est_us > 400.0) {
             struct timespec ts;
             const long ns = (long)(est_us * 750.0);
@@ -692,7 +720,7 @@
     const int kp = tc_list_len(k);
     if (!(flags & (VM_FLAG_FORCE_EXACT | VM_FLAG_FORCE_SIMT)) && kp)
         for (int nq = 64; nq >= 16; nq -= 16)
-            if (scan_tc_supported(s->dtype, s->dim, nq, kp)) return nq;
+            if (scan_tc_supported(s->scan_dtype(), s->dim, nq, kp)) return nq;
     return MAXQ;
 }
 
@@ -701,6 +729,7 @@
     vm_store *s = c.s;
     Workspace &w = s->ws;
     cudaStream_t st = c.st;
+    const int sdt = s->scan_dtype();
     const void *q_dev = c.queries;
     if (c.q_mem == VM_MEM_HOST) {
         const size_t qbytes = (size_t)c.nq * s->dim * dtype_size(c.q_dtype);
@@ -720,7 +749,7 @@
     if (!(c.flags & VM_FLAG_FORCE_EXACT) && s->size > 0) {
         int kp_tc = tc_list_len(c.k);
         int kp_simt = c.k <= 24 ? (c.k + 8 > 16 ? ((c.k + 8 + 7) & ~7) : 16) : 0;
-        bool tc_ok = kp_tc > 0 && scan_tc_supported(s->dtype, s->dim, c.nq, kp_tc);
+        bool tc_ok = kp_tc > 0 && scan_tc_supported(sdt, s->dim, c.nq, kp_tc);
         bool want_tc = !(c.flags & VM_FLAG_FORCE_SIMT);
         if (want_tc && tc_ok) { kernel = 2; kp = kp_tc; }
         else if (kp_simt > 0) { kernel = 1; kp = kp_simt; }
@@ -740,24 +769,25 @@
     }
 
     int nq_pad = kernel == 2 ? ((c.nq + 15) & ~15) : c.nq;
-    const int split = (kernel == 2 && s->dtype == VM_BF16 && !(c.flags & VM_FLAG_NO_SPLIT) &&
-                       (c.nq <= 48 || (c.flags & VM_FLAG_SPLIT)) && scan_tc_supported(s->dtype, s->dim, c.nq, kp, 1)) ? 1 : 0;
+    const int split = (kernel == 2 && sdt == VM_BF16 && !(c.flags & VM_FLAG_NO_SPLIT) &&
+                       (c.nq <= 48 || s->scan_shadowed() || (c.flags & VM_FLAG_SPLIT)) &&
+                       scan_tc_supported(sdt, s->dim, c.nq, kp, 1)) ? 1 : 0;
 #ifdef VIDMEM_NO_GRAPH_PDL
     const bool pdl = !(c.flags & (VM_FLAG_TIMING | FLAG_INTERNAL_CAPTURE));
 #else
     const bool pdl = !(c.flags & VM_FLAG_TIMING);
 #endif
     int rc = k_normalize_queries(q_dev, c.q_dtype, c.nq, nq_pad, s->dim, s->ld, (float *)w.q_f32.p,
-                                 (kernel == 2 && s->dtype == VM_BF16) ? w.q_bf16.p : nullptr,
+                                 (kernel == 2 && sdt == VM_BF16) ? w.q_bf16.p : nullptr,
                                  (int32_t *)w.flags.p + c.nq, kernel == 2 ? (uint32_t *)w.seed.p : nullptr,
-                                 kernel == 2 ? (int)(w.seed.bytes / 4) : 0, kernel == 2 && s->dtype == VM_F32, split, pdl, st);
+                                 kernel == 2 ? (int)(w.seed.bytes / 4) : 0, kernel == 2 && sdt == VM_F32, split, pdl, st);
     if (rc != VM_OK) return rc;
     ++launches;
-    const double eps = scan_eps(kernel, s->dtype, s->dim, split, s->rows_exact != nullptr);
+    const double eps = scan_eps(kernel, sdt, s->dim, split, s->scan_shadowed());
 
     ScanArgs a;
     ScanInfo sinfo;
-    a.rows = s->rows; a.inv_norms = s->inv_norms; a.dtype = s->dtype; a.n = s->size; a.dim = s->dim; a.ld = s->ld;
+    a.rows = s->scan_rows(); a.inv_norms = s->inv_norms; a.dtype = sdt; a.n = s->size; a.dim = s->dim; a.ld = s->ld;
     a.queries = (const float *)w.q_f32.p; a.nq = c.nq; a.kp = kp; a.cand = (uint64_t *)w.cand.p; a.stream = st;
     a.slab = (uint64_t *)w.cand.p; a.scnt = (int *)w.scnt.p;
     a.ubuf = (uint64_t *)w.ubuf.p; a.ucnt = (int *)w.seed.p + SEED_TAB_WORDS + 2 * MAXQ; a.ucap = SCAN_UNION_CAP;
@@ -783,7 +813,7 @@
                  (size_t)tiles * c.nq * SCAN_DUMP_TILE * 8 <= w.cand.bytes &&
                  select_rescore_fits((int)tiles, SCAN_DUMP_TILE, kp, s->exact_dtype(), s->dim, s->ld);
         s->last_band_ctas = a.dump ? 0 : a.ctas; s->last_band_nq = c.nq;
-        rc = launch_scan_tc(a, s->dtype == VM_BF16 ? w.q_bf16.p : w.q_f32.p, (uint32_t *)w.seed.p, (int *)w.flags.p + c.nq + 1, nullptr, &sinfo);
+        rc = launch_scan_tc(a, sdt == VM_BF16 ? w.q_bf16.p : w.q_f32.p, (uint32_t *)w.seed.p, (int *)w.flags.p + c.nq + 1, nullptr, &sinfo);
         launches += 1;
     }
     if (rc != VM_OK) return rc;
@@ -816,7 +846,7 @@
     auto run_collect = [&]() -> int {
         VM_CUDA_CHECK(cudaMemsetAsync(w.col_cnt.p, 0, (size_t)c.nq * 4, st));
         ScanCollect sc{(const float *)w.col_thr.p, (uint64_t *)w.col_buf.p, (int *)w.col_cnt.p, COLLECT_CAP, uncert};
-        int r = launch_scan_tc(a, s->dtype == VM_BF16 ? w.q_bf16.p : w.q_f32.p, nullptr, nullptr, &sc);
+        int r = launch_scan_tc(a, sdt == VM_BF16 ? w.q_bf16.p : w.q_f32.p, nullptr, nullptr, &sc);
         if (r != VM_OK) return r;
         return k_collect_rescore((const uint64_t *)w.col_buf.p, (const int *)w.col_cnt.p, COLLECT_CAP, rs, st);
     };
diff --git a/real-time-brain-inspired-video-memory_b200/csrc/pairs.cu b/real-time-brain-inspired-video-memory_b200/csrc/pairs.cu
--- a/real-time-brain-inspired-video-memory_b200/csrc/pairs.cu
+++ b/real-time-brain-inspired-video-memory_b200/csrc/pairs.cu
@@ -402,7 +402,7 @@
 }
 
 int k_row_inv_norms(const void *rows, int dtype, float *inv_norms, int64_t row0, int64_t n, int ld, int *extreme, cudaStream_t st,
-                    const double *exact = nullptr);
+                    const void *exact = nullptr, int exact_dtype = VM_F64);
 
 namespace {
 struct PairsWs {
diff --git a/real-time-brain-inspired-video-memory_b200/csrc/store.cu b/real-time-brain-inspired-video-memory_b200/csrc/store.cu
--- a/real-time-brain-inspired-video-memory_b200/csrc/store.cu
+++ b/real-time-brain-inspired-video-memory_b200/csrc/store.cu
@@ -24,7 +24,7 @@
 
 template <typename T>
 __global__ void row_inv_norms_kernel(const T *__restrict__ rows, float *__restrict__ inv_norms, int64_t row0,
-                                     int64_t n, int ld, int *__restrict__ extreme, const double *__restrict__ exact)
+                                     int64_t n, int ld, int *__restrict__ extreme, const void *__restrict__ exact, int exact_dtype)
 {
     int lane = threadIdx.x & 31;
     int64_t warp = (blockIdx.x * (int64_t)blockDim.x + threadIdx.x) >> 5;
@@ -39,8 +39,9 @@
         for (int o = 16; o > 0; o >>= 1) ss += __shfl_xor_sync(0xffffffffu, ss, o);
         double se = 0.0;
         if (exact != nullptr) {
+            const double scale = exact_dtype == VM_F64 ? 0x1p-600 : 1.0;
             for (int c = lane; c < ld; c += 32) {
-                const double v = exact[r * (int64_t)ld + c] * 0x1p-600;
+                const double v = load_as_double(exact, exact_dtype, r * (int64_t)ld + c) * scale;
                 se += v * v;
             }
             for (int o = 16; o > 0; o >>= 1) se += __shfl_xor_sync(0xffffffffu, se, o);
@@ -150,13 +151,16 @@
 }
 
 int k_row_inv_norms(const void *rows, int dtype, float *inv_norms, int64_t row0, int64_t n, int ld, int *extreme, cudaStream_t st,
-                    const double *exact)
+                    const void *exact, int exact_dtype)
 {
     if (n <= row0) return VM_OK;
     int64_t warps = n - row0;
     int grid = (int)vm::imin64((warps * 32 + 255) / 256, 148 * 16);
-    if (dtype == VM_F32) row_inv_norms_kernel<float><<<grid, 256, 0, st>>>((const float *)rows, inv_norms, row0, n, ld, extreme, exact);
-    else row_inv_norms_kernel<__nv_bfloat16><<<grid, 256, 0, st>>>((const __nv_bfloat16 *)rows, inv_norms, row0, n, ld, extreme, exact);
+    if (dtype == VM_F32)
+        row_inv_norms_kernel<float><<<grid, 256, 0, st>>>((const float *)rows, inv_norms, row0, n, ld, extreme, exact, exact_dtype);
+    else
+        row_inv_norms_kernel<__nv_bfloat16><<<grid, 256, 0, st>>>((const __nv_bfloat16 *)rows, inv_norms, row0, n, ld, extreme, exact,
+                                                                  exact_dtype);
     VM_CUDA_CHECK(cudaGetLastError());
     return VM_OK;
 }
diff --git a/real-time-brain-inspired-video-memory_b200/store.py b/real-time-brain-inspired-video-memory_b200/store.py
--- a/real-time-brain-inspired-video-memory_b200/store.py
+++ b/real-time-brain-inspired-video-memory_b200/store.py
@@ -42,7 +42,7 @@
 
 
 def device_row_limit(dim: int, dtype: str, device: int = 0) -> int:
-    per_row = ((int(dim) + 7) & ~7) * {"f32": 4, "bf16": 2, "f64+bf16": 10}.get(dtype, 12) + 4
+    per_row = ((int(dim) + 7) & ~7) * {"f32": 6, "bf16": 2, "f64+bf16": 10}.get(dtype, 12) + 4
     total = torch.cuda.get_device_properties(device).total_memory if torch.cuda.is_available() else 1 << 34
     return max(1, min(total // per_row, (1 << 31) - 512))
 
@@ -68,7 +68,8 @@
         self.dtype_code = _DT_EXACT[dtype] if self.exact else _DT[dtype]
         self.device = torch.device("cuda", device)
         self.ld = self.lib.vm_ld(self.dim)
-        self.rows_exact = None
+        self.rows_exact = self.rows_shadow = None
+        shadowed = not self.exact and self.dtype_code == L.VM_F32
         if self.growable:
             h = C.c_void_p()
             with torch.cuda.device(self.device):
@@ -86,14 +87,21 @@
             self.inv_norms = torch.empty((self.capacity,), dtype=torch.float32, device=self.device)
             if self.exact:
                 self.rows_exact = torch.empty((self.capacity, self.ld), dtype=torch.float64, device=self.device)
+            elif shadowed:
+                self.rows_shadow = torch.empty((self.capacity, self.ld), dtype=torch.bfloat16, device=self.device)
         elif self.exact:
             self.rows, self.inv_norms, self.rows_exact = _buffers
+        elif shadowed:
+            self.rows, self.inv_norms, self.rows_shadow = _buffers
         else:
             self.rows, self.inv_norms = _buffers
         h = C.c_void_p()
         if self.exact:
             L.check(self.lib.vm_store_attach_exact(C.byref(h), device, self.dim, self.dtype_code, self.capacity,
                                                    self.rows.data_ptr(), self.inv_norms.data_ptr(), self.rows_exact.data_ptr()))
+        elif shadowed:
+            L.check(self.lib.vm_store_attach_shadow(C.byref(h), device, self.dim, self.capacity, self.rows.data_ptr(),
+                                                    self.inv_norms.data_ptr(), self.rows_shadow.data_ptr()))
         else:
             L.check(self.lib.vm_store_attach(C.byref(h), device, self.dim, self.dtype_code, self.capacity,
                                              self.rows.data_ptr(), self.inv_norms.data_ptr()))
@@ -112,6 +120,9 @@
         self.inv_norms = torch.as_tensor(_DeviceRange(self.lib.vm_store_inv_norms_ptr(self._h), (cap,), "<f4"), device=dev)
         if self.exact:
             self.rows_exact = torch.as_tensor(_DeviceRange(self.lib.vm_store_rows_exact_ptr(self._h), (cap, self.ld), "<f8"), device=dev)
+        elif self.lib.vm_store_shadow_ptr(self._h):
+            self.rows_shadow = torch.as_tensor(_DeviceRange(self.lib.vm_store_shadow_ptr(self._h), (cap, self.ld), "<i2"),
+                                               device=dev).view(torch.bfloat16)
 
     def reserve(self, capacity: int) -> None:
         if int(capacity) <= self.capacity:
@@ -128,7 +139,8 @@
         n = int(n)
         if not 1 <= n <= len(self):
             raise ValueError(f"prefix of {n} rows outside [1, {len(self)}]")
-        bufs = (self.rows[:n], self.inv_norms[:n]) + ((self.rows_exact[:n],) if self.exact else ())
+        bufs = (self.rows[:n], self.inv_norms[:n]) + ((self.rows_exact[:n],) if self.exact else
+                                                       (self.rows_shadow[:n],) if self.rows_shadow is not None else ())
         v = EmbeddingStore(self.dim, n, self.dtype, self.device.index, _buffers=bufs)
         L.check(self.lib.vm_store_set_size(v._h, n, n, _stream_ptr(self.device)))
         return v
@@ -136,7 +148,7 @@
     def close(self) -> None:
         if getattr(self, "_h", None):
             if self.growable:
-                self.rows = self.inv_norms = self.rows_exact = None
+                self.rows = self.inv_norms = self.rows_exact = self.rows_shadow = None
             self.lib.vm_store_destroy(self._h)
             self._h = None
 
```

Result: faster. 438,700, median of 6 (+68.7%).
